# dkogan/horizonator

Measured on AMD Instinct MI355X. Metric: panorama Mpix/s (360deg, 16k-wide, 7x7 SRTM3 tiles), higher is better.
Workload: dtype f32

## Files before the change

### horizonator_amd/_lib.py

```python
import ctypes as C
import os

_HERE = os.path.dirname(os.path.abspath(__file__))
LIB_PATH = os.environ.get("HORIZONATOR_AMD_LIB") or os.path.join(_HERE, "libhorizonator.so")
DEMGEN_PATH = os.path.join(_HERE, "libhzdemgen.so")
SELFTEST_PATH = os.path.join(_HERE, "libhorizonator_selftest.so")

MAX_NDEMS_IJ = 4


class DemContext(C.Structure):
    _fields_ = [
        ("dems", (C.c_void_p * MAX_NDEMS_IJ) * MAX_NDEMS_IJ),
        ("mmap_sizes", (C.c_size_t * MAX_NDEMS_IJ) * MAX_NDEMS_IJ),
        ("mmap_fd", (C.c_int * MAX_NDEMS_IJ) * MAX_NDEMS_IJ),
        ("origin_dem_lon_lat", C.c_int * 2),
        ("origin_dem_cellij", C.c_int * 2),
        ("Ndems_ij", C.c_int * 2),
        ("radius_cells", C.c_int),
        ("cells_per_deg", C.c_int),
    ]


class _Offscreen(C.Structure):
    _fields_ = [
        ("inited", C.c_bool),
        ("frameBufID", C.c_uint32),
        ("renderBufID", C.c_uint32),
        ("depthBufID", C.c_uint32),
        ("width", C.c_int),
        ("height", C.c_int),
    ]


class Context(C.Structure):
    _fields_ = (
        [("Ntriangles", C.c_int), ("render_texture", C.c_bool), ("use_glut", C.c_bool),
         ("glut_window", C.c_int)]
        + [(name, C.c_int32) for name in (
            "uniform_aspect", "uniform_az_deg0", "uniform_az_deg1",
            "uniform_viewer_cell_i", "uniform_viewer_cell_j", "uniform_viewer_z",
            "uniform_viewer_lat", "uniform_cos_viewer_lat",
            "uniform_texturemap_lon0", "uniform_texturemap_lon1",
            "uniform_texturemap_dlat0", "uniform_texturemap_dlat1", "uniform_texturemap_dlat2",
            "uniform_znear", "uniform_zfar", "uniform_znear_color", "uniform_zfar_color")]
        + [("program", C.c_uint32), ("viewer_lat", C.c_float), ("viewer_lon", C.c_float),
           ("dems", DemContext), ("offscreen", _Offscreen)]
    )


class View(C.Structure):
    _fields_ = [(n, C.c_float) for n in (
        "viewer_cell_i", "viewer_cell_j", "viewer_z", "cos_viewer_lat", "deg_per_cell",
        "az_deg0", "az_deg1", "aspect", "znear", "zfar", "znear_color", "zfar_color")]


class Options(C.Structure):
    _fields_ = [(n, C.c_int) for n in (
        "serial", "rounds", "near_cells", "coarse_depth", "tiles", "tile_list", "adapt", "adapt_hi", "pretest_march",
        "worklists", "fast_math", "resolve_clears", "queue_capacity", "host_dense", "host_sectors", "host_times", "vertex_cache")]


class Times(C.Structure):
    _fields_ = [(n, C.c_float) for n in ("clear_ms", "raster_ms", "big_ms", "resolve_ms", "total_ms", "near_ms")]


class Window(C.Structure):
    _fields_ = [("cells_per_deg", C.c_int), ("radius_cells", C.c_int),
                ("origin_tile", C.c_int * 2), ("origin_cell", C.c_int * 2)]


class TexParams(C.Structure):
    _fields_ = [(n, C.c_float) for n in ("viewer_lat_rad", "origin_cell_lon_deg", "origin_cell_lat_deg",
                                         "lon0", "lon1", "dlat0", "dlat1", "dlat2")] + \
               [(n, C.c_int32) for n in ("ntiles_x", "ntiles_y", "lowest_x", "lowest_y", "tex_w", "tex_h")]


RASTER_AUTO, RASTER_SCATTER, RASTER_MARCH = 0, 1, 2

_lib = None
_selftest = None


def load():
    global _lib
    if _lib is None:
        _lib = _open(LIB_PATH, selftest=os.path.basename(LIB_PATH) == os.path.basename(SELFTEST_PATH))
    return _lib


def load_selftest():
    global _selftest
    if _selftest is None:
        _selftest = _open(SELFTEST_PATH, selftest=True)
    return _selftest


def _open(path, selftest):
    if not os.path.exists(path):
        raise ImportError(
            f"{path} is missing: build it with `make -C horizonator_amd/csrc` "
            "(or `python -c 'import __graft_entry__ as g; g.build()'`). "
            "horizonator_amd has no fallback implementation.")
    lib = C.CDLL(path, mode=C.RTLD_GLOBAL if not selftest else C.RTLD_LOCAL)
    P = C.POINTER
    ctxp = P(Context)
    f, i, b, d = C.c_float, C.c_int, C.c_bool, C.c_double
    vp = C.c_void_p

    def sig(name, res, *args):
        fn = getattr(lib, name)
        fn.restype = res
        fn.argtypes = list(args)

    sig("horizonator_init", b, ctxp, f, f, P(f), i, i, i, f, b, b, b,
        C.c_char_p, C.c_char_p, C.c_char_p, C.c_char_p, b)
    sig("horizonator_deinit", None, ctxp)
    sig("horizonator_resized", b, ctxp, i, i)
    sig("horizonator_pan_zoom", b, ctxp, f, f)
    sig("horizonator_move", b, ctxp, P(f), f, f)
    sig("horizonator_set_zextents", b, ctxp, f, f, f, f)
    sig("horizonator_redraw", b, ctxp)
    sig("horizonator_pick", b, ctxp, P(f), P(f), i, i)
    sig("horizonator_render_offscreen", b, ctxp, vp, vp)
    sig("horizonator_x_from_az", b, P(d), P(d), d, d, d, i)
    sig("horizonator_project", b, P(d), P(d), P(d), d, d, d, d, d, d, d, d, d, i, i)
    sig("horizonator_unproject", b, P(f), P(f), i, i, d, d, d, d, d, d, d, i, i)

    sig("horizonator_dem_init", b, P(DemContext), f, f, i, f, C.c_char_p, b)
    sig("horizonator_dem_deinit", None, P(DemContext))
    sig("horizonator_dem_sample", C.c_int16, P(DemContext), i, i)
    sig("horizonator_dem_bounds_latlon_deg", None, P(DemContext), P(f), P(f), P(f), P(f))

    sig("horizonator_amd_get_window", b, ctxp, P(Window))
    sig("horizonator_amd_init_from_mosaic", b, ctxp, f, f, P(f), i, i, P(Window), vp)
    sig("horizonator_amd_render", b, ctxp, vp, vp, vp, vp)
    sig("horizonator_amd_render_device", b, ctxp, vp, vp, vp, vp)
    sig("horizonator_amd_render_batch", b, ctxp, i, vp, vp, vp, vp, vp)
    sig("horizonator_amd_render_packed", b, ctxp, vp)
    sig("horizonator_amd_resolve_packed", b, ctxp, vp, i, i, i, vp, vp)
    sig("horizonator_amd_resolve_packed_strips", b, ctxp, i, vp, i, vp, vp, vp, vp)
    sig("horizonator_amd_render_sparse", b, ctxp, vp, i)
    sig("horizonator_amd_resolve_sparse_strips", b, ctxp, i, vp, i, vp, vp, vp, vp)
    sig("horizonator_amd_sync", b, ctxp)
    sig("horizonator_amd_texture_layout", b, ctxp, P(i), P(i), P(i), P(i))
    sig("horizonator_amd_set_texture", b, ctxp, vp)
    sig("horizonator_amd_set_sector", b, ctxp, i, i)
    sig("horizonator_amd_set_raster", b, ctxp, i)
    sig("horizonator_amd_set_profiling", b, ctxp, b)
    sig("horizonator_amd_render_begin", b, ctxp, vp, vp)
    sig("horizonator_amd_render_end", b, ctxp)
    sig("horizonator_amd_get_options", b, ctxp, P(Options))
    sig("horizonator_amd_set_options", b, ctxp, P(Options))
    sig("horizonator_amd_last_times", b, ctxp, P(Times))
    sig("horizonator_amd_get_view", b, ctxp, P(View))
    sig("horizonator_amd_device", vp, ctxp)
    sig("horizonator_amd_get_mosaic", b, ctxp, vp)
    sig("horizonator_amd_build_id", C.c_char_p)
    sig("horizonator_amd_link_cells_size", b, ctxp, i, i, i, P(i), P(i))
    sig("horizonator_amd_link_cells", b, ctxp, i, i, i, vp, vp)
    sig("horizonator_amd_poi_visibility", b, ctxp, i, vp, i, vp, vp, vp)

    sig("hz_hip_device_count", i)
    sig("hz_hip_create", vp, i, i, i, i)
    sig("hz_hip_destroy", None, vp)
    sig("hz_hip_upload_mosaic", i, vp, vp)
    sig("hz_hip_download_mosaic", i, vp, vp)
    sig("hz_hip_ingest_tiles", i, vp, vp, i, i, i, i, i)
    sig("hz_hip_set_sector", i, vp, i, i)
    sig("hz_hip_set_raster", i, vp, i)
    sig("hz_hip_set_profiling", i, vp, i)
    sig("hz_hip_get_options", i, vp, P(Options))
    sig("hz_hip_set_options", i, vp, P(Options))
    sig("hz_hip_set_texture", i, vp, P(TexParams), vp)
    sig("hz_hip_pack", i, vp, vp)
    sig("hz_hip_resolve_packed", i, vp, P(View), vp, vp, i, i, i, vp, vp)
    sig("hz_hip_pack_sparse", i, vp, vp, i)
    sig("hz_hip_resolve_sparse", i, vp, P(View), vp, vp, i, i, i, vp, vp)
    sig("hz_hip_resolve_sparse_strips", i, vp, P(View), vp, i, vp, i, vp, vp, vp, vp)
    sig("hz_hip_draw", i, vp, P(View))
    sig("hz_hip_resolve", i, vp, P(View), vp, vp, vp, vp, vp)
    sig("hz_hip_resolve_to_host", i, vp, P(View), vp, vp, vp, vp, vp)
    sig("hz_hip_render_to_host", i, vp, P(View), vp, vp, vp, vp, vp)
    sig("hz_hip_host_begin", i, vp, P(View), vp, vp, vp, vp, vp)
    sig("hz_hip_host_end", i, vp)
    sig("hz_hip_host_prepare", i, vp, i, i, i, i, vp)
    sig("hz_hip_read_depth", i, vp, i, i, P(C.c_uint32))
    sig("hz_hip_link_cells", i, vp, P(View), vp, vp, vp, vp, d, d, d, i, i, i, i, vp, vp)
    sig("hz_hip_poi_visibility", i, vp, P(View), vp, i, vp, i, vp, vp, vp)
    sig("hz_hip_sync", i, vp)
    sig("hz_hip_last_times", i, vp, P(Times))
    sig("hz_hip_stream", vp, vp)
    sig("hz_hip_wait_outputs", i, vp, vp)
    sig("hz_hip_wait_for", i, vp, vp)
    sig("horizonator_amd_stream_waits_for_outputs", b, ctxp, vp)
    sig("horizonator_amd_waits_for_stream", b, ctxp, vp)
    sig("hz_hip_last_plan", i, vp, vp)
    sig("hz_hip_last_queue_counts", i, vp, vp)
    sig("hz_hip_last_error", C.c_char_p)
    if selftest:
        sig("hz_hip_check_fastmath", i, i, i, C.c_uint64, C.c_uint64, P(C.c_uint64), vp)
        sig("hz_hip_check_exactness", i, i, i, C.c_uint64, C.c_uint64, i, i, i, i, P(C.c_uint64))
        sig("hz_hip_debug_bigqueue", i, vp, i, vp, i, vp)
        sig("hz_hip_debug_wave_timing", i, vp, P(View), vp, C.c_size_t, vp)
        sig("hz_hip_debug_worklist", C.c_long, i, i, i, P(View), i, i, i, vp, C.c_size_t)
    return lib


DECLARED_SYMBOLS = [
    "horizonator_init", "horizonator_deinit", "horizonator_resized", "horizonator_pan_zoom",
    "horizonator_move", "horizonator_set_zextents", "horizonator_redraw", "horizonator_pick",
    "horizonator_render_offscreen", "horizonator_x_from_az", "horizonator_project",
    "horizonator_unproject",
    "horizonator_dem_init", "horizonator_dem_deinit", "horizonator_dem_sample",
    "horizonator_dem_bounds_latlon_deg",
    "horizonator_amd_get_window", "horizonator_amd_init_from_mosaic",
    "horizonator_amd_render", "horizonator_amd_render_device", "horizonator_amd_render_batch",
    "horizonator_amd_render_packed", "horizonator_amd_resolve_packed",
    "horizonator_amd_resolve_packed_strips", "horizonator_amd_render_sparse",
    "horizonator_amd_resolve_sparse_strips",
    "horizonator_amd_sync", "horizonator_amd_stream_waits_for_outputs", "horizonator_amd_waits_for_stream", "horizonator_amd_texture_layout", "horizonator_amd_set_texture",
    "horizonator_amd_set_sector", "horizonator_amd_set_raster", "horizonator_amd_set_profiling",
    "horizonator_amd_get_options", "horizonator_amd_set_options", "horizonator_amd_render_begin", "horizonator_amd_render_end",
    "horizonator_amd_last_times", "horizonator_amd_get_view", "horizonator_amd_device",
    "horizonator_amd_get_mosaic", "horizonator_amd_link_cells_size", "horizonator_amd_link_cells",
    "horizonator_amd_poi_visibility", "horizonator_amd_build_id",
    "hz_hip_device_count", "hz_hip_create", "hz_hip_destroy", "hz_hip_upload_mosaic",
    "hz_hip_download_mosaic", "hz_hip_ingest_tiles", "hz_hip_set_sector", "hz_hip_set_raster",
    "hz_hip_set_profiling", "hz_hip_get_options", "hz_hip_set_options", "hz_hip_set_texture", "hz_hip_pack", "hz_hip_resolve_packed", "hz_hip_pack_sparse", "hz_hip_resolve_sparse", "hz_hip_resolve_sparse_strips", "hz_hip_draw", "hz_hip_resolve", "hz_hip_resolve_to_host", "hz_hip_render_to_host", "hz_hip_host_begin", "hz_hip_host_end", "hz_hip_host_prepare",
    "hz_hip_read_depth", "hz_hip_link_cells", "hz_hip_poi_visibility", "hz_hip_sync", "hz_hip_last_times", "hz_hip_stream", "hz_hip_wait_outputs", "hz_hip_wait_for", "hz_hip_last_plan", "hz_hip_last_queue_counts", "hz_hip_last_error",
]
SELFTEST_SYMBOLS = ["hz_hip_check_fastmath", "hz_hip_check_exactness", "hz_hip_debug_bigqueue", "hz_hip_debug_wave_timing",
                    "hz_hip_debug_worklist"]


def load_demgen():
    if not os.path.exists(DEMGEN_PATH):
        raise ImportError(f"{DEMGEN_PATH} is missing: build it with `make -C horizonator_amd/csrc`")
    lib = C.CDLL(DEMGEN_PATH)
    lib.hz_demgen_write_region.restype = C.c_int
    lib.hz_demgen_write_region.argtypes = [C.c_char_p] + [C.c_int] * 6
    lib.hz_demgen_write_tile.restype = C.c_int
    lib.hz_demgen_write_tile.argtypes = [C.c_char_p] + [C.c_int] * 4
    lib.hz_demgen_tile_values.restype = None
    lib.hz_demgen_tile_values.argtypes = [C.c_void_p] + [C.c_int] * 4
    return lib
```

### horizonator_amd/csrc/hz_context.cpp

```cpp
#include "hz_dev.h"

#include <time.h>

thread_local char hz_g_last_error[512];
extern "C" const char* hz_hip_last_error(void) { return g_last_error; }


static int env_int(const char* name, int dflt) { const char* e = getenv(name); return e ? atoi(e) : dflt; }
static hz_options_t default_options(void)
{
    hz_options_t o;
    o.serial         = 0;
    o.rounds         = 0;
    o.near_cells     = -1;
    o.coarse_depth   = -1;
    o.tiles          = -1;
    o.tile_list      = 0;
    o.adapt          = 1;
    o.adapt_hi       = -1;
    o.pretest_march  = -1;
    o.worklists      = 1;
    o.fast_math      = 1;
    o.resolve_clears = 1;
    o.queue_capacity = 0;
    o.host_dense     = 0;
    o.host_sectors   = 0;
    o.host_times     = 0;
    o.vertex_cache   = 1;
    return o;
}
hz_options_t hz_options_from_env(void)
{
    hz_options_t o = default_options();
    o.serial         = env_int("HZ_SERIAL", o.serial) != 0;
    if(getenv("HZ_TWO_PASS")) o.rounds = env_int("HZ_TWO_PASS", 0) != 0 ? 2 : 1;
    o.near_cells     = env_int("HZ_NEAR_CELLS", o.near_cells);
    if(getenv("HZ_HIZ")) o.coarse_depth = env_int("HZ_HIZ", 0) != 0;
    o.tiles          = env_int("HZ_TILES", o.tiles);
    o.tile_list      = env_int("HZ_TILE_LIST", o.tile_list);
    o.adapt          = env_int("HZ_ADAPT", o.adapt);
    o.adapt_hi       = env_int("HZ_ADAPT_HI", o.adapt_hi);
    if(getenv("HZ_PRETEST_MARCH")) o.pretest_march = env_int("HZ_PRETEST_MARCH", 0) != 0;
    o.worklists      = env_int("HZ_NO_WORKLIST", 0) == 0;
    o.fast_math      = env_int("HZ_NO_FAST_MATH", 0) == 0;
    o.resolve_clears = env_int("HZ_RESOLVE_CLEARS", o.resolve_clears) != 0;
    o.queue_capacity = env_int("HZ_QUEUE_CAPACITY", o.queue_capacity);
    o.host_dense     = env_int("HZ_HOST_DENSE", o.host_dense) != 0;
    o.host_sectors   = env_int("HZ_HOST_SECTORS", o.host_sectors);
    o.host_times     = env_int("HZ_HOST_TIMES", o.host_times) != 0;
    o.vertex_cache   = env_int("HZ_VERTEX_CACHE", o.vertex_cache) != 0;
    return o;
}
#ifdef HZ_EXPERIMENTS
static hz_experiments_t experiments_from_env(void)
{
    hz_experiments_t e = { env_int("HZ_MARCH_DEBUG", 0), env_int("HZ_EXP_FB_MARCH", 0), env_int("HZ_EXP_FB_BIG", 0) };
    return e;
}
#endif
extern "C" int hz_hip_device_count(void)
{
    int n = 0;
    if(hipGetDeviceCount(&n) != hipSuccess) return 0;
    return n;
}

hipError_t hz_sync_all(hz_dev_t* d)
{
    hipError_t rc = hipSuccess;
    hipStream_t all[4] = { d->stream, d->nstream, d->qstream, d->rstream };
    for(int k=0; k<4; k++)
        if(all[k]) { const hipError_t e = hipStreamSynchronize(all[k]); if(e != hipSuccess) rc = e; }
    return rc;
}

extern "C" void hz_hip_destroy(hz_dev_t* d)
{
    if(!d) return;
    hz_device_guard device_guard_(d->device);
    (void)hz_sync_all(d);
    (void)hipFree(d->d_mosaic);
    for(int i=0; i<HZ_NFB; i++) { (void)hipFree(d->d_fbs[i]); (void)hipFree(d->d_touched[i]); }
    for(int i=0; i<2*HZ_NFB; i++)
    {
        (void)hipFree(d->d_bigrec_s[i]);
        (void)hipFree(d->d_bigitem_s[i]);
        (void)hipFree(d->d_midrec_s[i]);
        (void)hipFree(d->d_clip_s[i]);
        (void)hipFree(d->d_big_counters_s[i]);
        (void)hipFree(d->tiles_s[i].cursor); (void)hipFree(d->tiles_s[i].pairs); (void)hipFree(d->tiles_s[i].state); (void)hipFree(d->tiles_s[i].busy);
    }
    if(d->ev_marched) (void)hipEventDestroy(d->ev_marched);
    if(d->ev_near)    (void)hipEventDestroy(d->ev_near);
    for(int i=0; i<HZ_NFB; i++) (void)hipFree(d->d_hiz[i]);
    for(int c=0; c<HZ_LIST_CACHE; c++)
        for(int k=0; k<HZ_NLISTS; k++)
        {
            hz_worklists_t& wl = d->list_cache[c];
            (void)hipFree(wl.d_items[k]);
            for(int t=0; t<2; t++)
            {
                if(wl.h_items[k][t])   (void)hipHostFree(wl.h_items[k][t]);
                if(wl.ev_copied[k][t]) (void)hipEventDestroy(wl.ev_copied[k][t]);
            }
        }
    delete d->list_scratch; delete d->list_scratch2;
    (void)hipFree(d->d_texels);
    (void)hipFree(d->d_tanel);
    free(d->h_tanel);
    hz_hostpath_destroy(d);
    (void)hipFree(d->vc.d_polar);
    if(d->vc.ev_filled) (void)hipEventDestroy(d->vc.ev_filled);
    for(int k=0; k<10; k++) if(d->ev[k]) (void)hipEventDestroy(d->ev[k]);
    for(int k=0; k<HZ_NFB; k++) { if(d->adapt.ev[k]) (void)hipEventDestroy(d->adapt.ev[k]); if(d->adapt.h_counts[k]) (void)hipHostFree(d->adapt.h_counts[k]); }
    if(d->ev_drawn)   (void)hipEventDestroy(d->ev_drawn);
    for(int i=0; i<HZ_NFB; i++) if(d->ev_free[i]) (void)hipEventDestroy(d->ev_free[i]);
    if(d->ev_readers) (void)hipEventDestroy(d->ev_readers);
    if(d->ev_tanel)   (void)hipEventDestroy(d->ev_tanel);
    if(d->rstream && d->rstream != d->stream) (void)hipStreamDestroy(d->rstream);
    if(d->qstream && d->qstream != d->stream) (void)hipStreamDestroy(d->qstream);
    if(d->nstream && d->nstream != d->stream) (void)hipStreamDestroy(d->nstream);

    if(d->stream) (void)hipStreamDestroy(d->stream);
    free(d);
}

int hz_tile_bins(hz_dev_t* d, int set)
{
    tl_bins_t& tb = d->tiles_s[set];
    if(tb.cursor) return 0;
    if(d->tiles_unavailable) return 1;
    const size_t ntiles = (size_t)((d->W + TL_W-1)/TL_W)*((d->H + TL_H-1)/TL_H);
    hipError_t e = hipMalloc(&tb.pairs, ntiles*TL_LIST*sizeof(unsigned int));
    if(e == hipSuccess) e = hipMalloc(&tb.state, 2*sizeof(unsigned int));
    if(e == hipSuccess) e = hipMalloc(&tb.busy, TL_UNITS_PER_TILE*ntiles*sizeof(unsigned int));
    if(e == hipSuccess) e = hipMalloc(&tb.cursor, ntiles*sizeof(unsigned int));
    if(e != hipSuccess)
    {
        (void)hipGetLastError();
        (void)hipFree(tb.pairs); (void)hipFree(tb.state); (void)hipFree(tb.busy); (void)hipFree(tb.cursor);
        tb.pairs = tb.state = tb.busy = tb.cursor = NULL;
        d->tiles_unavailable = 1;
        return 1;
    }
    return 0;
}

mr_queue_t hz_queue_set(const hz_dev_t* d, int k)
{
    const bool first_round = k >= HZ_NFB;
    mr_queue_t q = { d->d_bigrec_s[k], d->d_bigitem_s[k], d->d_midrec_s[k], d->d_clip_s[k], d->d_big_counters_s[k],
                     first_round ? d->near_bigrec_capacity  : d->bigrec_capacity,
                     first_round ? d->near_bigitem_capacity : d->bigitem_capacity,
                     first_round ? 0u : d->midrec_capacity,
                     first_round ? d->near_clip_capacity : d->clip_capacity };
    return q;
}


static int create_impl(hz_dev_t* d)
{
    hz_stopwatch sw("HZ_INIT_TIMES");
    HZ_ON_DEVICE(d);
    sw.lap("first HIP call (runtime, device)");
    d->env = hz_options_from_env();
#ifdef HZ_EXPERIMENTS
    d->exp = experiments_from_env();
#endif
    d->list_scratch = new std::vector<uint32_t>();
    d->list_scratch2 = new std::vector<uint32_t>();
    d->lists = &d->list_cache[0];
    HZ_CHECK(hipStreamCreateWithFlags(&d->stream, hipStreamNonBlocking));
    if(d->env.serial) d->rstream = d->stream;
    else HZ_CHECK(hipStreamCreateWithFlags(&d->rstream, hipStreamNonBlocking));
    HZ_CHECK(hipEventCreateWithFlags(&d->ev_drawn,   hipEventDisableTiming));
    for(int i=0; i<HZ_NFB; i++) HZ_CHECK(hipEventCreateWithFlags(&d->ev_free[i], hipEventDisableTiming));
    HZ_CHECK(hipEventCreateWithFlags(&d->ev_readers, hipEventDisableTiming));
    HZ_CHECK(hipEventCreateWithFlags(&d->ev_tanel,   hipEventDisableTiming));
    HZ_CHECK(hipMalloc(&d->d_mosaic, (size_t)d->N*d->N*sizeof(int16_t)));
    sw.lap("streams, events, mosaic");
    d->seg_stride = (d->W + HZ_SEG-1) / HZ_SEG;
    for(int i=0; i<HZ_NFB; i++)
    {
        HZ_CHECK(hipMalloc(&d->d_fbs[i], (size_t)d->W*d->H*sizeof(unsigned long long)));
        HZ_CHECK(hipMemsetAsync(d->d_fbs[i], 0xFF, (size_t)d->W*d->H*sizeof(unsigned long long), d->rstream));
        HZ_CHECK(hipMalloc(&d->d_touched[i], (size_t)d->seg_stride*d->H));
        HZ_CHECK(hipMemsetAsync(d->d_touched[i], 0, (size_t)d->seg_stride*d->H, d->rstream));
        HZ_CHECK(hipEventRecord(d->ev_free[i], d->rstream));
        d->fb_used[i] = 0;
    }
    d->fbi = HZ_NFB-1; d->d_fb = d->d_fbs[HZ_NFB-1];
    sw.lap("framebuffers");
    {
        const size_t per16 = (size_t)d->W*d->H/16;
        unsigned int rec = per16 > (1u<<24) ? (1u<<24) : per16 < (1u<<15) ? (1u<<15) : (unsigned int)per16;
        d->bigrec_capacity  = rec;
        d->bigitem_capacity = 2*rec;
        d->midrec_capacity  = rec;
        d->clip_capacity    = rec;
        const size_t r = (size_t)(d->env.near_cells > HZ_NEAR_CELLS_MAX ? d->env.near_cells : HZ_NEAR_CELLS_MAX);
        const size_t near_tris = 2*(2*r + 2)*(2*r + 2*MR_COLS);
        d->near_bigrec_capacity  = near_tris < rec ? (unsigned int)near_tris : rec;
        d->near_bigitem_capacity = 2*rec;
        d->near_clip_capacity    = d->near_bigrec_capacity;
        if(d->env.queue_capacity > 0)
            d->bigrec_capacity = d->bigitem_capacity = d->midrec_capacity = d->clip_capacity =
            d->near_bigrec_capacity = d->near_bigitem_capacity = d->near_clip_capacity = (unsigned int)d->env.queue_capacity;
    }
    if(d->env.serial) d->qstream = d->nstream = d->stream;
    else
    {
        HZ_CHECK(hipStreamCreateWithFlags(&d->qstream, hipStreamNonBlocking));
        HZ_CHECK(hipStreamCreateWithFlags(&d->nstream, hipStreamNonBlocking));
    }
    HZ_CHECK(hipEventCreateWithFlags(&d->ev_marched, hipEventDisableTiming));
    HZ_CHECK(hipEventCreateWithFlags(&d->ev_near,    hipEventDisableTiming));
    for(int i=0; i<2*HZ_NFB; i++)
    {
        const mr_queue_t q = hz_queue_set(d, i);
        HZ_CHECK(hipMalloc(&d->d_bigrec_s[i],  (size_t)q.bigrec_capacity*sizeof(hz_bigrec_t)));
        HZ_CHECK(hipMalloc(&d->d_bigitem_s[i], (size_t)q.bigitem_capacity*sizeof(hz_bigitem_t)));
        if(q.midrec_capacity) HZ_CHECK(hipMalloc(&d->d_midrec_s[i], (size_t)q.midrec_capacity*sizeof(hz_rec_t)));
        HZ_CHECK(hipMalloc(&d->d_clip_s[i],    (size_t)q.clip_capacity*sizeof(uint32_t)));
        HZ_CHECK(hipMalloc(&d->d_big_counters_s[i], HZ_NCOUNTERS*sizeof(unsigned int)));
        HZ_CHECK(hipMemset(d->d_big_counters_s[i], 0, HZ_NCOUNTERS*sizeof(unsigned int)));
        if(d->env.tiles > 0 && i >= HZ_NFB && hz_tile_bins(d, i) != 0) return -1;
    }
    sw.lap("queue sets");
    HZ_CHECK(hipEventRecord(d->ev_drawn, d->qstream));
    HZ_CHECK(hipMalloc(&d->d_tanel, (size_t)d->H*sizeof(float)));
    d->h_tanel = (float*)malloc((size_t)d->H*sizeof(float));
    d->tanel_resident = 0;
    for(int k=0; k<10; k++) HZ_CHECK(hipEventCreate(&d->ev[k]));
    for(int k=0; k<HZ_NFB; k++)
    {
        HZ_CHECK(hipHostMalloc((void**)&d->adapt.h_counts[k], 6*sizeof(unsigned int), hipHostMallocDefault));
        HZ_CHECK(hipEventCreateWithFlags(&d->adapt.ev[k], hipEventDisableTiming | hipEventReleaseToSystem));
    }
    sw.lap("the rest");
    return 0;
}

extern "C" hz_dev_t* hz_hip_create(int device, int N, int width, int height)
{
    if(N < 2 || width <= 0 || height <= 0)
    {
        snprintf(g_last_error, sizeof(g_last_error), "hz_hip_create: bad sizes N=%d W=%d H=%d", N, width, height);
        return NULL;
    }
    if((unsigned long long)width*(unsigned long long)height >= (1ull << 29))
    {
        snprintf(g_last_error, sizeof(g_last_error), "hz_hip_create: images of up to 2^29 pixels (%d x %d asked for)", width, height);
        fprintf(stderr, "hz_hip: %s\n", g_last_error);
        return NULL;
    }
    hz_dev_t* d = (hz_dev_t*)calloc(1, sizeof(*d));
    if(!d) return NULL;
    d->device = device; d->N = N; d->W = width; d->H = height;
    d->col0 = 0; d->col1 = width;
    d->raster = HZ_RASTER_AUTO;
    if(create_impl(d) != 0) { hz_hip_destroy(d); return NULL; }
    return d;
}

extern "C" int hz_hip_upload_mosaic(hz_dev_t* d, const int16_t* mosaic)
{
    HZ_ON_DEVICE(d);
    HZ_CHECK(hz_sync_all(d));
    HZ_CHECK(hipMemcpyAsync(d->d_mosaic, mosaic, (size_t)d->N*d->N*sizeof(int16_t), hipMemcpyHostToDevice, d->stream));
    HZ_CHECK(hipStreamSynchronize(d->stream));
    d->adapt.have_view = 0;
    d->vc.state = 0;
    return 0;
}

extern "C" int hz_hip_download_mosaic(hz_dev_t* d, int16_t* mosaic)
{
    HZ_ON_DEVICE(d);
    HZ_CHECK(hipMemcpyAsync(mosaic, d->d_mosaic, (size_t)d->N*d->N*sizeof(int16_t), hipMemcpyDeviceToHost, d->stream));
    HZ_CHECK(hipStreamSynchronize(d->stream));
    return 0;
}


extern "C" int hz_hip_set_sector(hz_dev_t* d, int col0, int col1)
{
    if(col0 < 0 || col1 > d->W || col0 >= col1)
    {
        snprintf(g_last_error, sizeof(g_last_error), "hz_hip_set_sector: bad sector [%d,%d) of %d", col0, col1, d->W);
        return -1;
    }
    d->col0 = col0; d->col1 = col1;
    return 0;
}

extern "C" int hz_hip_set_raster(hz_dev_t* d, int which)
{
    if(which < HZ_RASTER_AUTO || which > HZ_RASTER_MARCH) return -1;
    d->raster = which;
    return 0;
}

extern "C" int hz_hip_set_texture(hz_dev_t* d, const hz_texparams_t* params, const unsigned char* texels_bgr)
{
    HZ_ON_DEVICE(d);
    if(params == NULL) { d->tex_on = 0; return 0; }
    if(params->tex_w <= 0 || params->tex_h <= 0 || params->ntiles_x <= 0 || params->ntiles_y <= 0)
    {
        snprintf(g_last_error, sizeof(g_last_error), "hz_hip_set_texture: empty texture");
        return -1;
    }
    if(texels_bgr != NULL)
    {
        const size_t n = (size_t)params->tex_w*params->tex_h;
        uint32_t* packed = (uint32_t*)malloc(n*sizeof(uint32_t));
        if(!packed) { snprintf(g_last_error, sizeof(g_last_error), "hz_hip_set_texture: out of memory"); return -1; }
        for(size_t k=0; k<n; k++)
            packed[k] = (uint32_t)texels_bgr[3*k] | ((uint32_t)texels_bgr[3*k+1] << 8) | ((uint32_t)texels_bgr[3*k+2] << 16);
        HZ_CHECK(hipStreamSynchronize(d->stream));
        HZ_CHECK(hipStreamSynchronize(d->rstream));
        (void)hipFree(d->d_texels); d->d_texels = NULL;
        hipError_t e = hipMalloc(&d->d_texels, n*sizeof(uint32_t));
        if(e == hipSuccess) e = hipMemcpy(d->d_texels, packed, n*sizeof(uint32_t), hipMemcpyHostToDevice);
        free(packed);
        HZ_CHECK(e);
    }
    else if(d->d_texels == NULL || params->tex_w != d->tex.tex_w || params->tex_h != d->tex.tex_h)
    {
        snprintf(g_last_error, sizeof(g_last_error), "hz_hip_set_texture: no texture of that size is resident");
        return -1;
    }
    d->tex = *params;
    d->tex_on = 1;
    return 0;
}

extern "C" int hz_hip_set_profiling(hz_dev_t* d, int on) { d->profiling = on; return 0; }

extern "C" int hz_hip_get_options(hz_dev_t* d, hz_options_t* o)
{
    if(!d || !o) return -1;
    *o = d->env;
    return 0;
}
extern "C" int hz_hip_set_options(hz_dev_t* d, const hz_options_t* o)
{
    if(!d || !o) return -1;
    HZ_ON_DEVICE(d);
    HZ_CHECK(hz_sync_all(d));
    const int serial = d->env.serial, queue_capacity = d->env.queue_capacity;
    d->env = *o;
    d->env.serial = serial; d->env.queue_capacity = queue_capacity;
    for(int c=0; c<HZ_LIST_CACHE; c++) d->list_cache[c].valid = 0;
    d->adapt.have_view = 0;
    return 0;
}
extern "C" void* hz_hip_stream(hz_dev_t* d) { return (void*)d->rstream; }

extern "C" int hz_hip_wait_outputs(hz_dev_t* d, void* stream)
{
    HZ_ON_DEVICE(d);
    HZ_CHECK(hipEventRecord(d->ev_tanel, d->rstream));
    HZ_CHECK(hipStreamWaitEvent((hipStream_t)stream, d->ev_tanel, 0));
    return 0;
}

extern "C" int hz_hip_wait_for(hz_dev_t* d, void* stream)
{
    HZ_ON_DEVICE(d);
    HZ_CHECK(hipEventRecord(d->ev_tanel, (hipStream_t)stream));
    HZ_CHECK(hipStreamWaitEvent(d->rstream, d->ev_tanel, 0));
    return 0;
}

extern "C" int hz_hip_last_queue_counts(hz_dev_t* d, unsigned int* out)
{
    if(!d || !out) return -1;
    out[0] = (unsigned int)d->adapt.seen_reach; out[1] = d->adapt.seen_records; out[2] = d->adapt.seen_items; out[3] = (unsigned int)d->adapt.long_reach;
    return 0;
}

extern "C" int hz_hip_last_plan(hz_dev_t* d, int* out)
{
    if(!d || !out) return -1;
    for(int k=0; k<5; k++) out[k] = d->last_plan[k];
    return 0;
}


extern "C" int hz_hip_sync(hz_dev_t* d)
{
    HZ_ON_DEVICE(d);
    HZ_CHECK(hz_sync_all(d));
    return 0;
}

extern "C" int hz_hip_last_times(hz_dev_t* d, hz_times_t* t)
{
    memset(t, 0, sizeof(*t));
    if(!d->have_times) return -1;
    HZ_ON_DEVICE(d);
    HZ_CHECK(hz_sync_all(d));
    HZ_CHECK(hipEventElapsedTime(&t->clear_ms,  d->ev[0], d->ev[1]));
    HZ_CHECK(hipEventElapsedTime(&t->near_ms,   d->ev[7], d->ev[6]));
    HZ_CHECK(hipEventElapsedTime(&t->raster_ms, d->ev[9], d->ev[2]));
    HZ_CHECK(hipEventElapsedTime(&t->big_ms,    d->ev[8], d->ev[3]));
    if(d->have_times == 2)
        HZ_CHECK(hipEventElapsedTime(&t->resolve_ms, d->ev[4], d->ev[5]));
    t->total_ms = t->clear_ms + t->near_ms + t->raster_ms + t->big_ms + t->resolve_ms;
    return 0;
}
```

### horizonator_amd/csrc/hz_dev.h

```cpp
#pragma once

#include <hip/hip_runtime_api.h>

#include <math.h>
#include <stdio.h>
#include <stdlib.h>
#include <string.h>
#include <time.h>

#include <vector>

#include "hz_hip.h"
#include "hz_types.h"
#include "hz_launch.h"


extern thread_local char hz_g_last_error[512];
#define g_last_error hz_g_last_error

#define HZ_CHECK(call)                                                        \
    do {                                                                      \
        hipError_t e_ = (call);                                               \
        if(e_ != hipSuccess)                                                  \
        {                                                                     \
            snprintf(g_last_error, sizeof(g_last_error), "%s:%d %s -> %s",    \
                     __FILE__, __LINE__, #call, hipGetErrorString(e_));       \
            fprintf(stderr, "hz_hip: %s\n", g_last_error);                    \
            return -1;                                                        \
        }                                                                     \
    } while(0)

struct hz_device_guard
{
    int prev, dev; bool ok;
    explicit hz_device_guard(int device) : prev(-1), dev(device), ok(true)
    {
        if(hipGetDevice(&prev) != hipSuccess) prev = -1;
        if(prev != dev)
        {
            const hipError_t e = hipSetDevice(dev);
            if(e != hipSuccess)
            {
                ok = false;
                snprintf(g_last_error, sizeof(g_last_error), "hipSetDevice(%d) -> %s", dev, hipGetErrorString(e));
                fprintf(stderr, "hz_hip: %s\n", g_last_error);
            }
        }
    }
    ~hz_device_guard() { if(ok && prev >= 0 && prev != dev) (void)hipSetDevice(prev); }
};
#define HZ_ON_DEVICE(d) hz_device_guard device_guard_((d)->device); if(!device_guard_.ok) return -1

#ifdef HZ_EXPERIMENTS
struct hz_experiments_t { int march_debug, exp_fb_march, exp_fb_big; };
#endif

struct hz_listkey_t
{
    hz_view_t view; int col0, col1, two_pass, near_x0, near_x1, near_j0, near_j1, far_rows;
};
#define HZ_NLISTS 2
struct hz_worklists_t
{
    uint32_t*    d_items[HZ_NLISTS];
    uint32_t*    h_items[HZ_NLISTS][2];
    size_t       cap[HZ_NLISTS];
    unsigned int n[HZ_NLISTS];
    hipEvent_t   ev_copied[HZ_NLISTS][2];
    int          turn[HZ_NLISTS];
    int          valid;
    unsigned int last_used;
    hz_listkey_t key;
};
#define HZ_LIST_CACHE 8

struct hz_dev
{
    int device;
    hz_options_t env;
#ifdef HZ_EXPERIMENTS
    hz_experiments_t exp;
#endif
    int N, W, H;
    int col0, col1;
    int raster;
    int profiling;
    hz_worklists_t list_cache[HZ_LIST_CACHE];
    hz_worklists_t* lists;
    unsigned int lists_clock;
    std::vector<uint32_t>* list_scratch;
    std::vector<uint32_t>* list_scratch2;
    struct { unsigned long long* d_cycles; size_t capacity; unsigned int grid_x, grid_y; } wave_timing;

    hipStream_t stream, rstream;
    hipEvent_t  ev_drawn, ev_free[HZ_NFB], ev_readers, ev_tanel;
    int16_t*            d_mosaic;
    unsigned long long* d_fbs[HZ_NFB];
    size_t              fb_used[HZ_NFB];
    int                 fbi;
    unsigned long long* d_fb;
    unsigned char*      d_touched[HZ_NFB];
    int                 seg_stride;
    hipStream_t         qstream, nstream;
    hipEvent_t          ev_marched, ev_near;
    uint32_t*           d_hiz[HZ_NFB];
    int                 hiz_unavailable;
    int                 tiles_unavailable;
    struct
    {
        unsigned int* h_counts[HZ_NFB];
        hipEvent_t    ev[HZ_NFB];
        int           pending[HZ_NFB], long_of[HZ_NFB], reach_of[HZ_NFB];
        unsigned int  serial_of[HZ_NFB];
        hz_view_t     view; int col0, col1, have_view;
        unsigned int  serial;
        unsigned int  items_short;
        int           tried_long;
        int           long_reach;
        int           seen_reach; unsigned int seen_records, seen_items;
    } adapt;
    struct { hz_polar_t* d_polar; hz_xform_t key; int state ; int unavailable; hipEvent_t ev_filled;
             int same_draw;      } vc;
    int                 last_qshards_log2;
    int                 last_plan[5];
    int                 stream_reads_fb;
    hz_bigrec_t*        d_bigrec_s[2*HZ_NFB];
    hz_bigitem_t*       d_bigitem_s[2*HZ_NFB];
    hz_rec_t*           d_midrec_s[2*HZ_NFB];
    uint32_t*           d_clip_s[2*HZ_NFB];
    unsigned int*       d_big_counters_s[2*HZ_NFB];
    unsigned int        bigrec_capacity, bigitem_capacity, midrec_capacity, clip_capacity;
    unsigned int        near_bigrec_capacity, near_bigitem_capacity, near_clip_capacity;
    tl_bins_t           tiles_s[2*HZ_NFB];
    hz_view_t           last_view;
    int                 have_view;
    int                 fb_consumed;
    float*              d_tanel;
    float*              h_tanel;
    int                 tanel_resident;

    struct hz_hoststate* host;

    uint32_t*      d_texels;
    hz_texparams_t tex;
    int            tex_on;

    hipEvent_t ev[10];
    int        have_times;
    hz_times_t times;
};

#define HZ_NEAR_PX            20.0f
#define HZ_TWO_ROUNDS_MIN_PIX 6.0e6
#define HZ_TILES_MIN_PX       35.0f
#define HZ_HIZ_MIN_PX         25.0f



struct hz_stopwatch
{
    bool on; timespec t0;
    explicit hz_stopwatch(const char* var) : on(getenv(var) && atoi(getenv(var)) != 0) { clock_gettime(CLOCK_MONOTONIC, &t0); }
    void lap(const char* what)
    {
        if(!on) return;
        timespec t1; clock_gettime(CLOCK_MONOTONIC, &t1);
        fprintf(stderr, "hz_hip init: %-34s %8.2f ms\n", what, 1e3*(double)(t1.tv_sec - t0.tv_sec) + 1e-6*(double)(t1.tv_nsec - t0.tv_nsec));
        t0 = t1;
    }
};


hz_options_t hz_options_from_env(void);
mr_queue_t   hz_queue_set(const hz_dev_t* d, int k);
int          hz_tile_bins(hz_dev_t* d, int set);
hipError_t   hz_sync_all(hz_dev_t* d);
hz_params_t  hz_make_params(const hz_dev_t* d, const hz_view_t* v);
int          hz_plan_rounds(const hz_dev_t* d, const hz_view_t* view, hz_params_t& p);
mr_zones_t   hz_make_zones(const hz_params_t& p, bool near_first);
bool         hz_azimuths_of_columns(const hz_params_t& p, double* a0, double* a1);
void         hz_list_items(const hz_params_t& p, const mr_zones_t& zn, double a0, double a1, std::vector<uint32_t>& out, bool every_strip = false);
void         hz_list_rounds(const hz_params_t& p, const mr_zones_t& zn, double a0, double a1, bool one_round,
                            std::vector<uint32_t>* first, std::vector<uint32_t>& second, bool every_strip = false);
int          hz_draw_impl(hz_dev_t* d, const hz_view_t* view);
int          hz_fb_refill(hz_dev_t* d);
int          hz_fb_mark_consumed(hz_dev_t* d);
int          hz_upload_tanel(hz_dev_t* d, const float* tanel);
int          hz_rstream_after_draw(hz_dev_t* d);
int          hz_resolve_impl(hz_dev_t* d, const hz_view_t* view, const float* tanel,
                             unsigned char* bgr, float* ranges, int32_t* index, uint32_t* z24, int nbands, hipEvent_t* ev_band, int* band_rows);
void         hz_hostpath_destroy(hz_dev_t* d);
int          hz_gpu_numa_node(const hz_dev_t* d);
void         hz_hostpath_landing(hz_dev_t* d, unsigned char** pinned, size_t* bytes);
```

### horizonator_amd/csrc/hz_fast.h

```cpp
#pragma once

#include "hz_num.h"

#ifdef __HIPCC__

#define HZF_LO 9.31322575e-10f
#define HZF_HI 1073741824.0f

__device__ static inline int hzf_in_range(float x) { const float a = hz_abs(x); return a >= HZF_LO && a <= HZF_HI; }

__device__ static inline float hzf_refined_rcp(float c)
{
    const float r = __builtin_amdgcn_rcpf(c);
    const float e = __builtin_fmaf(-c, r, 1.0f);
    return __builtin_fmaf(e, r, r);
}
__device__ static inline float hzf_div_by(float a, float c, float rr)
{
    float q = a*rr;
    float e = __builtin_fmaf(-c, q, a);
    q = __builtin_fmaf(e, rr, q);
    e = __builtin_fmaf(-c, q, a);
    return __builtin_fmaf(e, rr, q);
}
__device__ static inline float hzf_div(float a, float b) { return hzf_div_by(a, b, hzf_refined_rcp(b)); }
__device__ static inline float hzf_rcp(float b)          { return hzf_refined_rcp(b); }
__device__ static inline float hzf_div_by_two_pi(float a, float rr)
{
    const float q = a*rr;
    const float e = __builtin_fmaf(-HZ_TWO_PI, q, a);
    return __builtin_fmaf(e, rr, q);
}
__device__ static inline float hzf_fold_to_unit(float t) { return (1.0f < t) ? hzf_rcp(t) : t; }

__device__ static inline float hzf_sqrt(float x)
{
    const float y = __builtin_amdgcn_rsqf(x);
    const float s = x*y;
    const float h = 0.5f*y;
    const float r = __builtin_fmaf(-s, s, x);
    return __builtin_fmaf(r, h, s);
}

typedef struct { float rr_two_pi, rr_zrange, rr_crange, zrange, crange; } hzf_const_t;

__device__ static inline hzf_const_t hzf_setup(const hz_xform_t* u)
{
    hzf_const_t c;
    c.zrange = u->zfar - u->znear;
    c.crange = u->zfar_color - u->znear_color;
    float two_pi = HZ_TWO_PI;
    asm volatile("" : "+v"(two_pi));
    c.rr_two_pi = hzf_refined_rcp(two_pi);
    c.rr_zrange = hzf_refined_rcp(c.zrange);
    c.rr_crange = hzf_refined_rcp(c.crange);
    return c;
}

template<bool XPOS>
__device__ static inline float hzf_atan2_r(float y, float x, float rcp)
{
    const bool  flip = XPOS ? false : (0.f >= x);
    const float ax   = hz_abs(x);
    const float s    = flip ? ax : y;
    const float sot  = s * rcp;
    const float tn   = (ax == hz_abs(y)) ? 1.0f : hz_abs(sot);

    const float u  = hzf_fold_to_unit(tn);
    const float u2 = u*u;
    const float u3 = u2*u;
    const float u5 = u3*u2;
    const float u7 = u5*u2;
    const float u9 = u7*u2;
    float p = u*0.9999793128310355f + u3*-0.3326756418091246f;
    p = p + u5*0.1938924977115610f;
    p = p + u7*-0.1173503194786851f;
    p = p + u9*0.0536813784310406f;
    p = p + (u9*-0.0121323213173444f)*u2;
    const float a   = (1.0f < tn) ? ((p*-2.0f + HZ_HALF_PI) + p) : p;
    const float arc = flip ? (HZ_HALF_PI + a) : a;
    const uint32_t sign = ((uint32_t)__float_as_int(y) | (uint32_t)__float_as_int(rcp)) & 0x80000000u;
    return __int_as_float((int)((uint32_t)__float_as_int(arc) | sign));
}
template<bool XPOS>
__device__ static inline float hzf_atan2(float y, float x)
{
    const float t = (XPOS ? false : (0.f >= x)) ? y : hz_abs(x);
    return hzf_atan2_r<XPOS>(y, x, hzf_rcp(t));
}

__device__ static inline hz_polar_t hzf_polar_en_r(const hz_xform_t* u, float e, float n, float fz, float rcp_az)
{
    hz_polar_t q;
    const float h = fz - u->viewer_z;
    const float nn = n*n, ee = e*e;
    q.d_ne  = hzf_sqrt(nn + ee);
    q.az    = hzf_atan2_r<false>(e, n, rcp_az);
    q.el    = hzf_atan2<true>(h, q.d_ne);
    q.d_enh = hzf_sqrt(h*h + nn + ee);
    return q;
}
__device__ static inline hz_polar_t hzf_polar_en(const hz_xform_t* u, float e, float n, float fz)
{
    return hzf_polar_en_r(u, e, n, fz, hzf_rcp((0.f >= n) ? e : hz_abs(n)));
}
__device__ static inline hz_vertex_t hzf_finish(const hz_xform_t* u, const hzf_const_t* c, hz_polar_t q)
{
    hz_vertex_t v;
    const float d = hzf_div_by_two_pi(q.az + -u->az_center, c->rr_two_pi);
    v.x = (HZ_TWO_PI*(d - hz_roundeven(d))) * u->az_ndc_per_rad;
    v.y = q.el * u->aspect * u->az_ndc_per_rad;
    v.z = hzf_div_by(q.d_enh - u->znear, c->zrange, c->rr_zrange) * 2.0f + -1.0f;

    const float r = hzf_div_by(q.d_ne - u->znear_color, c->crange, c->rr_crange);
    v.red = hz_min(hz_max(r, 0.0f), 1.0f);
    return v;
}
__device__ static inline hz_vertex_t hzf_transform_en(const hz_xform_t* u, const hzf_const_t* c, float e, float n, float fz)
{
    return hzf_finish(u, c, hzf_polar_en(u, e, n, fz));
}
__device__ static inline hz_vertex_t hzf_transform_en_r(const hz_xform_t* u, const hzf_const_t* c, float e, float n, float fz, float rcp_az)
{
    return hzf_finish(u, c, hzf_polar_en_r(u, e, n, fz, rcp_az));
}

#endif

HZ_HD int hzf_draw_ok(const hz_xform_t* u)
{
    const float lo = 9.31322575e-10f, hi = 1073741824.0f;
    const float vz = hz_abs(u->viewer_z), ce = hz_abs(u->az_center);
    const float zr = hz_abs(u->zfar - u->znear), cr = hz_abs(u->zfar_color - u->znear_color);
    if(!(vz == 0.0f || (vz >= 0.015625f && vz <= 536870912.0f))) return 0;
    if(!(ce == 0.0f || (ce >= 8.8817842e-16f && ce <= 1048576.0f))) return 0;
    if(!(u->znear >= lo && u->znear <= hi && hz_abs(u->zfar) >= lo && hz_abs(u->zfar) <= hi && zr >= lo && zr <= hi)) return 0;
    if(!(hz_abs(u->znear_color) >= lo && hz_abs(u->znear_color) <= hi &&
         hz_abs(u->zfar_color) >= lo && hz_abs(u->zfar_color) <= hi && cr >= lo && cr <= hi)) return 0;
    if(!(hz_abs(u->aspect) <= hi && hz_abs(u->az_ndc_per_rad) <= hi)) return 0;
    return 1;
}
```

### horizonator_amd/csrc/hz_ingest.cpp

```cpp
#include "hz_dev.h"
#include "hz_pool.h"

extern "C" int hz_hip_ingest_tiles(hz_dev_t* d, const unsigned char* const* tiles,
                                   int ntx, int nty, int cpd, int oc_x, int oc_y)
{
    HZ_ON_DEVICE(d);
    const int nt = ntx*nty;
    const size_t tile_bytes = (size_t)(cpd+1)*(cpd+1)*2;
    if(nt <= 0 || !tiles) { snprintf(g_last_error, sizeof(g_last_error), "hz_hip_ingest_tiles: no tiles"); return -1; }
    HZ_CHECK(hz_sync_all(d));
    int npresent = 0;
    for(int k=0; k<nt; k++) if(tiles[k]) npresent++;
    unsigned char* d_raw = NULL;
    unsigned char** d_ptrs = NULL;
    unsigned char* own_stage = NULL;
    std::vector<unsigned char*> h_ptrs((size_t)nt, (unsigned char*)NULL);
    int rc = -1;
    hipEvent_t ev[3] = { NULL, NULL, NULL };
    do {
        if(npresent && hipMalloc(&d_raw, (size_t)npresent*tile_bytes) != hipSuccess) { snprintf(g_last_error, sizeof(g_last_error), "hz_hip_ingest_tiles: no device memory for %d tiles", npresent); break; }
        if(hipMalloc(&d_ptrs, (size_t)nt*sizeof(*d_ptrs)) != hipSuccess) break;
        for(int k=0, at=0; k<nt; k++) if(tiles[k]) h_ptrs[(size_t)k] = d_raw + (size_t)(at++)*tile_bytes;
        unsigned char* stage = NULL; size_t stage_bytes = 0;
        hz_hostpath_landing(d, &stage, &stage_bytes);
        if(stage_bytes < ((size_t)3 << 20))
        {
            stage_bytes = (size_t)24 << 20;
            if(hipHostMalloc((void**)&own_stage, stage_bytes, hipHostMallocDefault) != hipSuccess) { snprintf(g_last_error, sizeof(g_last_error), "hz_hip_ingest_tiles: no pinned memory"); break; }
            stage = own_stage;
        }
        size_t piece = stage_bytes/3 & ~(size_t)4095;
        if(piece > ((size_t)64 << 20)) piece = (size_t)64 << 20;
        bool ok = true;
        for(int k=0; k<3 && ok; k++) ok = hipEventCreateWithFlags(&ev[k], hipEventDisableTiming) == hipSuccess;
        if(!ok) break;
        hz_copy_pool* pool = copy_pool(hz_gpu_numa_node(d));
        const size_t total = (size_t)npresent*tile_bytes;
        std::vector<const unsigned char*> src;
        for(int k=0; k<nt; k++) if(tiles[k]) src.push_back(tiles[k]);
        size_t turn = 0;
        for(size_t off = 0; off < total && ok; off += piece, turn++)
        {
            const size_t n = total - off < piece ? total - off : piece;
            unsigned char* buf = stage + (turn % 3)*piece;
            if(turn >= 3) ok = hipEventSynchronize(ev[turn % 3]) == hipSuccess;
            if(!ok) break;
            hz_copy_pool::batch_t copied = { 0 };
            for(size_t o = off; o < off + n; )
            {
                const size_t t = o/tile_bytes, in = o - t*tile_bytes;
                const size_t len = tile_bytes - in < off + n - o ? tile_bytes - in : off + n - o;
                pool->push(&copied, buf + (o - off), src[t] + in, len, (size_t)1 << 20);
                o += len;
            }
            pool->wait(&copied);
            ok = hipMemcpyAsync(d_raw + off, buf, n, hipMemcpyHostToDevice, d->stream) == hipSuccess
              && hipEventRecord(ev[turn % 3], d->stream) == hipSuccess;
        }
        if(!ok) { snprintf(g_last_error, sizeof(g_last_error), "hz_hip_ingest_tiles: tile upload failed"); break; }
        if(hipMemcpyAsync(d_ptrs, h_ptrs.data(), (size_t)nt*sizeof(*d_ptrs), hipMemcpyHostToDevice, d->stream) != hipSuccess) break;
        dim3 grid((d->N + 255)/256, d->N);
        hzk_ingest(grid, dim3(256), d->stream, (const unsigned char* const*)d_ptrs, d->d_mosaic, d->N, ntx, nty, cpd, oc_x, oc_y);
        if(hipGetLastError() != hipSuccess) break;
        if(hipStreamSynchronize(d->stream) != hipSuccess) break;
        d->adapt.have_view = 0;
        d->vc.state = 0;
        rc = 0;
    } while(0);
    (void)hipStreamSynchronize(d->stream);
    for(int k=0; k<3; k++) if(ev[k]) (void)hipEventDestroy(ev[k]);
    (void)hipFree(d_raw); (void)hipFree(d_ptrs);
    if(own_stage) (void)hipHostFree(own_stage);
    (void)hipGetLastError();
    return rc;
}
```

### horizonator_amd/csrc/hz_k_march.h

```cpp
#pragma once


#define MR_CAP    128
#define MR_RSLOTS 4
#define MR_FIELDS 6

struct mr_lds_t
{
    uint32_t rows[MR_RSLOTS][MR_FIELDS][64];
    uint32_t ids[MR_CAP];
    uint32_t clip[64];
    uint32_t nclip;
};

__device__ static inline void mr_clip_flush(mr_lds_t& L, const mr_queue_t& q, int lane)
{
    const unsigned int nclip = (unsigned int)__builtin_amdgcn_readfirstlane((int)L.nclip);
    if(!nclip) return;
    uint32_t base = 0;
    if(lane == 0) base = atomicAdd(&q.counters[4], nclip);
    base = (uint32_t)__builtin_amdgcn_readfirstlane((int)base);
    if((unsigned int)lane < nclip)
    {
        const uint32_t at = base + (uint32_t)lane;
        if(at < q.clip_capacity) q.clip[at] = L.clip[lane];
    }
    __syncthreads();
    if(lane == 0) L.nclip = 0;
    __syncthreads();
}
__device__ static inline void mr_clip_note(mr_lds_t& L, const mr_queue_t& q, bool want, uint32_t prim, int lane)
{
    const unsigned long long m = __ballot(want);
    if(!m) return;
    const unsigned int n = (unsigned int)__popcll(m);
    unsigned int nclip = (unsigned int)__builtin_amdgcn_readfirstlane((int)L.nclip);
    if(nclip + n > 64u) { mr_clip_flush(L, q, lane); nclip = 0; }
    if(want) L.clip[nclip + (unsigned int)__popcll(m & ((1ull << lane) - 1ull))] = prim;
    __syncthreads();
    if(lane == 0) L.nclip = nclip + n;
    __syncthreads();
}

__device__ static inline void mr_store_row(mr_lds_t& L, int slot, int lane, const hz_wvert_t& v)
{
    L.rows[slot][0][lane] = __float_as_uint(v.wx);  L.rows[slot][1][lane] = __float_as_uint(v.wy);
    L.rows[slot][2][lane] = __float_as_uint(v.zw);  L.rows[slot][3][lane] = __float_as_uint(v.red);
    L.rows[slot][4][lane] = (uint32_t)v.xs;         L.rows[slot][5][lane] = (uint32_t)v.ys;
}
__device__ static inline hz_wvert_t mr_load_vert(const mr_lds_t& L, int slot, int lane)
{
    hz_wvert_t v;
    v.xn  = 0.f;
    v.wx  = __uint_as_float(L.rows[slot][0][lane]); v.wy  = __uint_as_float(L.rows[slot][1][lane]);
    v.zw  = __uint_as_float(L.rows[slot][2][lane]); v.red = __uint_as_float(L.rows[slot][3][lane]);
    v.xs  = (int32_t)L.rows[slot][4][lane];         v.ys  = (int32_t)L.rows[slot][5][lane];
    v.cmask = 0;
    return v;
}

__device__ static inline hz_wvert_t mr_load_vert_pos(const mr_lds_t& L, int slot, int lane)
{
    hz_wvert_t v;
    v.xn  = 0.f; v.red = 0.f; v.cmask = 0;
    v.wx  = __uint_as_float(L.rows[slot][0][lane]); v.wy  = __uint_as_float(L.rows[slot][1][lane]);
    v.zw  = __uint_as_float(L.rows[slot][2][lane]);
    v.xs  = (int32_t)L.rows[slot][4][lane];         v.ys  = (int32_t)L.rows[slot][5][lane];
    return v;
}


__device__ static inline int32_t mr_from_east(int32_t v)
{
    return __builtin_amdgcn_update_dpp(0, v, 0x130 , 0xF, 0xF, true);
}
__device__ static inline float mr_from_east(float v)
{
    return __int_as_float(__builtin_amdgcn_update_dpp(0, __float_as_int(v), 0x130, 0xF, 0xF, true));
}



__device__ static inline int32_t hz_imin(int32_t a, int32_t b) { return a < b ? a : b; }
__device__ static inline int32_t hz_imax(int32_t a, int32_t b) { return a > b ? a : b; }

struct mr_rowstate_t
{
    float    xn;
    int32_t  xs, ys;
    uint32_t cmask;
    uint32_t c, f1;
    uint32_t e_c, e_f1;
    uint32_t h_c, h_f1;
    int32_t  h_dx, h_dy;
};

__device__ static inline hz_wvert_t mr_window(const hz_vertex_t& vtx, const hz_params_t& p, bool* in_volume, bool* in_guard)
{
    hz_wvert_t cur;
    cur.xn  = vtx.x;
    cur.wx  = vtx.x*p.halfW + p.halfW;
    cur.wy  = vtx.y*p.halfH + p.halfH;
    cur.zw  = vtx.z*0.5f + 0.5f;
    cur.red = vtx.red;
    const float fxw = cur.wx - 0.5f, fyw = cur.wy - 0.5f;
    *in_guard  = hz_abs(fxw) <= HZ_GUARD_PX && hz_abs(fyw) <= HZ_GUARD_PX;
    *in_volume = __builtin_fmaxf(__builtin_fmaxf(hz_abs(vtx.x), hz_abs(vtx.y)), hz_abs(vtx.z)) <= 1.0f;
    cur.xs = (int32_t)hz_roundeven(fxw*256.f);
    cur.ys = (int32_t)hz_roundeven(fyw*256.f);
    cur.cmask = 0;
    return cur;
}
__device__ static inline void mr_window_flags(hz_wvert_t& cur, const hz_vertex_t& vtx, bool in_guard)
{
    cur.cmask = hz_clip_mask(vtx.x, vtx.y, vtx.z);
    if(!in_guard) { cur.xs = HZ_OUTSIDE_GUARD; cur.ys = 0; }
}

__device__ static inline uint32_t mr_pk_min(uint32_t a, uint32_t b)
{
    typedef unsigned short u16x2 __attribute__((ext_vector_type(2)));
    return __builtin_bit_cast(uint32_t, __builtin_elementwise_min(__builtin_bit_cast(u16x2, a), __builtin_bit_cast(u16x2, b)));
}
__device__ static inline uint32_t mr_pk_max(uint32_t a, uint32_t b)
{
    typedef unsigned short u16x2 __attribute__((ext_vector_type(2)));
    return __builtin_bit_cast(uint32_t, __builtin_elementwise_max(__builtin_bit_cast(u16x2, a), __builtin_bit_cast(u16x2, b)));
}
__device__ static inline bool mr_pk_lt(uint32_t a, uint32_t b)
{
    typedef unsigned short u16x2 __attribute__((ext_vector_type(2)));
    const u16x2 x = __builtin_bit_cast(u16x2, a), y = __builtin_bit_cast(u16x2, b);
    return x.x < y.x && x.y < y.y;
}
__device__ static inline uint32_t mr_from_east_u(uint32_t v) { return (uint32_t)mr_from_east((int32_t)v); }

__device__ static inline mr_rowstate_t mr_rowstate_of(const hz_wvert_t& cur, const hz_params_t& p)
{
    mr_rowstate_t now;
    now.xn = cur.xn; now.xs = cur.xs; now.ys = cur.ys; now.cmask = cur.cmask;
    const uint32_t c_x  = (uint32_t)((cur.xs + (HZ_SUBPIXEL_ONE-1)) >> HZ_SUBPIXEL_BITS), c_y  = (uint32_t)((cur.ys + (HZ_SUBPIXEL_ONE-1)) >> HZ_SUBPIXEL_BITS);
    const uint32_t f1_x = (uint32_t)((cur.xs + HZ_SUBPIXEL_ONE) >> HZ_SUBPIXEL_BITS),     f1_y = (uint32_t)((cur.ys + HZ_SUBPIXEL_ONE) >> HZ_SUBPIXEL_BITS);
    now.c  = mr_pk_max(c_x  | (c_y  << 16), (uint32_t)p.col0);
    now.f1 = mr_pk_min(f1_x | (f1_y << 16), (uint32_t)p.col1 | ((uint32_t)p.H << 16));
    now.e_c  = mr_from_east_u(now.c);
    now.e_f1 = mr_from_east_u(now.f1);
    now.h_c  = mr_pk_min(now.e_c,  now.c);
    now.h_f1 = mr_pk_max(now.e_f1, now.f1);
    now.h_dx = (int32_t)((uint32_t)mr_from_east(cur.xs) - (uint32_t)cur.xs);
    now.h_dy = (int32_t)((uint32_t)mr_from_east(cur.ys) - (uint32_t)cur.ys);
    return now;
}

__device__ static inline bool mr_simple_cull(const mr_rowstate_t& prev, const mr_rowstate_t& now, bool has_cell,
                                             const hz_params_t& p, bool* keep0, bool* keep1)
{
    const int32_t d01x = (int32_t)((uint32_t)now.xs - (uint32_t)prev.xs);
    const int32_t d01y = (int32_t)((uint32_t)now.ys - (uint32_t)prev.ys);
    const int32_t d11x = (int32_t)((uint32_t)d01x + (uint32_t)now.h_dx);
    const int32_t d11y = (int32_t)((uint32_t)d01y + (uint32_t)now.h_dy);
    const int32_t d10x = prev.h_dx, d10y = prev.h_dy;
    const int32_t lo = hz_imin(hz_imin(d01x, d11x), d10x), hi = hz_imax(hz_imax(d01x, d11x), d10x);
    if(__any(has_cell && !(lo > -p.quad_max_dx && hi < p.quad_max_dx))) return false;
    const int64_t area0 = (int64_t)d11x*(int64_t)d01y - (int64_t)d01x*(int64_t)d11y;
    const int64_t area1 = (int64_t)d10x*(int64_t)d11y - (int64_t)d11x*(int64_t)d10y;
    const uint32_t c0 = mr_pk_min(now.h_c, prev.c),                 f0 = mr_pk_max(now.h_f1, prev.f1);
    const uint32_t c1 = mr_pk_min(now.e_c, prev.h_c), f1 = mr_pk_max(now.e_f1, prev.h_f1);
    const bool box0 = mr_pk_lt(c0, f0), box1 = mr_pk_lt(c1, f1);
    *keep0 = has_cell && area0 > 0 && box0;
    *keep1 = has_cell && area1 > 0 && box1;
    return true;
}

__device__ static void mr_distribute(const hz_rec_t& r, uint32_t npix, int lane,
                                     unsigned long long* fb, const hz_params_t& p)
{
    uint32_t done = 0;
    for(;;)
    {
        const bool more = npix > done;
        if(__popcll(__ballot(more)) < 32) break;
        if(more)
        {
            const int ry = (int)(((float)done + 0.5f) * r.inv_bw);
            const int rx = (int)done - ry*r.bw;
            hz_emit_rec<false>(fb, p, r, r.px0 + rx, r.py0 + ry);
            done++;
        }
    }

    const uint32_t rest  = npix > done ? npix - done : 0;
    const uint32_t incl  = mr_scan(rest, lane);
    const uint32_t excl  = incl - rest;
    const uint32_t total = (uint32_t)__builtin_amdgcn_readlane((int)incl, 63);
    for(uint32_t base = 0; base < total; base += 64)
    {
        const uint32_t it = base + lane;
        int lo = 0;
        #pragma unroll
        for(int step=32; step>=1; step>>=1)
        {
            const uint32_t v = __shfl(excl, lo + step);
            if(v <= it) lo += step;
        }
        hz_rec_t o;
        #pragma unroll
        for(int m=0; m<3; m++)
        {
            o.e.dx[m]  = __shfl(r.e.dx[m], lo);  o.e.ndy[m] = __shfl(r.e.ndy[m], lo);
            o.e.glo[m] = __shfl(r.e.glo[m], lo); o.e.ghi[m] = __shfl(r.e.ghi[m], lo);
        }
        o.z_org = __shfl(r.z_org, lo); o.dzdx = __shfl(r.dzdx, lo); o.dzdy = __shfl(r.dzdy, lo);
        o.r_org = __shfl(r.r_org, lo); o.drdx = __shfl(r.drdx, lo); o.drdy = __shfl(r.drdy, lo);
        o.px0 = __shfl(r.px0, lo); o.py0 = __shfl(r.py0, lo); o.bw = __shfl(r.bw, lo);
        o.inv_bw = __shfl(r.inv_bw, lo);
        o.prim = __shfl(r.prim, lo);
        const uint32_t oexcl = __shfl(excl, lo), odone = __shfl(done, lo);
        if(it < total)
        {
            const uint32_t local = it - oexcl + odone;
            const int ry = (int)(((float)local + 0.5f) * o.inv_bw);
            const int rx = (int)local - ry*o.bw;
            hz_emit_rec<false>(fb, p, o, o.px0 + rx, o.py0 + ry);
        }
    }
}

__global__ __launch_bounds__(64)
void k_mid(unsigned long long* __restrict__ fb, const hz_rec_t* __restrict__ midrec,
           const unsigned int* __restrict__ counters, unsigned int midrec_capacity, hz_params_t p)
{
    const int lane = threadIdx.x;
    const int sl = p.qshards_log2;
    unsigned int longest = 0;
    #pragma unroll
    for(int s=0; s<HZ_QSHARDS; s++) { const unsigned int* c = hz_qshard(counters, s) + 4; longest = max(longest, min(min(c[0], ~c[1]), HZ_QSHARD_ROOM(midrec_capacity, sl))); }
    const unsigned int n = ((longest + HZ_QBLOCK-1) & ~(unsigned int)(HZ_QBLOCK-1)) << sl;
    for(unsigned int base = blockIdx.x*64u; base < n; base += gridDim.x*64u)
    {
        hz_rec_t r = {};
        uint32_t npix = 0;
        const unsigned int g = base + lane, block = g >> HZ_QBLOCK_LOG2;
        const unsigned int* c = hz_qshard(counters, (int)(block & ((1u << sl) - 1u))) + 4;
        if(g < n && (((block >> sl) << HZ_QBLOCK_LOG2) | (g & (HZ_QBLOCK-1))) < min(min(c[0], ~c[1]), HZ_QSHARD_ROOM(midrec_capacity, sl)))
        {
            r = midrec[g];
            npix = __float_as_uint(r.inv_bw);
            r.inv_bw = 1.0f / (float)r.bw;
        }
        mr_distribute(r, npix, lane, fb, p);
    }
}

template<bool HIZ, bool SHARDS>
__device__ static void mr_flush(const mr_lds_t& L, unsigned int head, unsigned int n, int lane,
                                int jbeg, int i0,
                                unsigned long long* fb, const mr_queue_t& q, const hz_params_t& p,
                                unsigned int* dbg = nullptr)
{
    hz_rec_t r;
    uint32_t npix = 0;
    int bh = 0;
    bool live = (unsigned int)lane < n;
    const bool valid = live;
    const uint32_t id_own = L.ids[(head + lane) & (MR_CAP-1)];
    const uint32_t id = valid ? id_own : (uint32_t)__builtin_amdgcn_readlane((int)id_own, 0);
    const int t = id & 1, l = (id >> 1) & 63, rowoff = id >> 7;
    const int s0 = rowoff & (MR_RSLOTS-1), s1 = (rowoff+1) & (MR_RSLOTS-1);
    const int sa = s0,               la = l;
    const int sb = t == 0 ? s1 : s0, lb = l+1;
    const int sc = s1,               lc = t == 0 ? l : l+1;
    hz_wvert_t a = mr_load_vert_pos(L, sa, la);
    hz_wvert_t b = mr_load_vert_pos(L, sb, lb);
    hz_wvert_t c = mr_load_vert_pos(L, sc, lc);
    hz_box_t box;
    hz_tri_box(&box, &a, &b, &c, p.col0, p.col1-1, 0, p.H-1);
    if(p.early_z)
    {
        if(valid && box.px1 - box.px0 <= 3 && box.py1 - box.py0 <= 1)
        {
            const char* hi = (const char*)fb + 4;
            const uint32_t rowbytes = (uint32_t)p.SW*8u;
            const uint32_t o0 = (uint32_t)box.py0*rowbytes, o1 = box.py1 > box.py0 ? o0 + rowbytes : o0;
            const int c0 = box.px0 - p.col0, cl = box.px1 - p.col0;
            typedef uint32_t u3_t __attribute__((ext_vector_type(3)));
            const int ca = min(c0, p.SW - 2), cb = min(max(cl - 1, c0), p.SW - 2);
            const uint32_t ba = 8u*(uint32_t)ca, bb = 8u*(uint32_t)cb;
            const u3_t a0 = *(const u3_t*)(hi + (o0 + ba)), b0 = *(const u3_t*)(hi + (o0 + bb));
            const u3_t a1 = *(const u3_t*)(hi + (o1 + ba)), b1 = *(const u3_t*)(hi + (o1 + bb));
            const uint32_t zs = max(max(max(a0.x, a0.z), max(b0.x, b0.z)), max(max(a1.x, a1.z), max(b1.x, b1.z))) >> 8;
            if(hz_tri_hidden(&a, &b, &c, p.z_hide_k, zs)) live = false;
        }
        else if(HIZ && valid && p.hiz)
        {
            const int bw1 = box.px1 - box.px0, bh1 = box.py1 - box.py0;
            const bool lv1 = bw1 <= (1 << HIZ1_W_LOG2) && bh1 <= (1 << HIZ1_H_LOG2);
            if(lv1 || (bw1 <= (1 << HIZ2_W_LOG2) && bh1 <= (1 << HIZ2_H_LOG2)))
            {
                const uint32_t* t = lv1 ? p.hiz : hiz_level2(p);
                const int sx = lv1 ? HIZ1_W_LOG2 : HIZ2_W_LOG2, sy = lv1 ? HIZ1_H_LOG2 : HIZ2_H_LOG2;
                const uint32_t tw = (uint32_t)(lv1 ? hiz_w1(p.SW) : hiz_w2(p.SW));
                const uint32_t tx0 = (uint32_t)(box.px0 - p.col0) >> sx, tx1 = (uint32_t)(box.px1 - p.col0) >> sx;
                const uint32_t o0 = ((uint32_t)box.py0 >> sy)*tw, o1 = ((uint32_t)box.py1 >> sy)*tw;
                const uint32_t z00 = t[o0 + tx0], z01 = t[o0 + tx1], z10 = t[o1 + tx0], z11 = t[o1 + tx1];
                const uint32_t zs = max(max(z00, z01), max(z10, z11)) >> 8;
                if(hz_tri_hidden(&a, &b, &c, p.z_hide_k, zs)) live = false;
            }
        }
        if(dbg) { dbg[5] += (unsigned int)__popcll(__ballot(valid && !live)); }
        if(HZ_DEBUG(p) == 2) return;
        if(!__any(live))
        {
            if(dbg) { dbg[0] += 1; dbg[1] += n; }
            return;
        }
    }
    {
        a.red = __uint_as_float(L.rows[sa][3][la]);
        b.red = __uint_as_float(L.rows[sb][3][lb]);
        c.red = __uint_as_float(L.rows[sc][3][lc]);
        hz_tri_t tri;
        hz_tri_planes(&tri, &a, &b, &c);
        hz_rec_from_tri(r, tri);
        r.px0 = box.px0; r.bw = box.px1 - box.px0 + 1;
        r.py0 = box.py0; bh   = box.py1 - box.py0 + 1;
        r.prim = (uint32_t)(((size_t)(jbeg + rowoff)*(p.N-1) + (i0 + l))*2 + t);
        npix = live ? (uint32_t)r.bw*(uint32_t)bh : 0u;
        r.inv_bw = __all(npix <= 64u) ? __builtin_amdgcn_rcpf((float)r.bw) : 1.0f / (float)r.bw;
    }

    const bool is_big = live && npix > p.big_min;
    const unsigned long long bigmask = __ballot(is_big);
    if(dbg) { dbg[0] += 1; dbg[1] += n; dbg[2] += (unsigned int)__popcll(bigmask); }
    const unsigned long long t_app0 = (dbg && HZ_DEBUG(p) == 4) ? __builtin_amdgcn_s_memtime() : 0ull;
    if(bigmask)
    {
        uint32_t chunks = 0;
        if(is_big)
        {
            chunks = hz_big_chunks(r.bw, bh);
        }
        const uint32_t incl  = mr_scan(chunks, lane);
        const uint32_t total = (uint32_t)__builtin_amdgcn_readlane((int)incl, 63);
        const uint32_t nb    = (uint32_t)__popcll(bigmask);
        uint32_t rbase = 0, ibase = 0, ok = 0;
        const int sl = SHARDS ? HZ_QSHARDS_LOG2 : 0, shard = (int)((blockIdx.x + 5u*blockIdx.y) & ((1u << sl) - 1u));
        if(lane == 0)
        {
            ok = hz_queue_reserve(q, shard, sl, nb, total, &rbase, &ibase) ? 1u : 0u;
        }
        rbase = (uint32_t)__builtin_amdgcn_readfirstlane((int)rbase); ibase = (uint32_t)__builtin_amdgcn_readfirstlane((int)ibase); ok = (uint32_t)__builtin_amdgcn_readfirstlane((int)ok);
        if(is_big)
        {
            if(ok)
            {
                const uint32_t ri = HZ_QSLOT(rbase + (uint32_t)__popcll(bigmask & ((1ull << lane) - 1ull)), shard, sl);
                const uint32_t ii = ibase + (incl - chunks);
                q.bigrec[ri].r = r; q.bigrec[ri].bh = bh;
                for(uint32_t c2=0; c2<chunks; c2++) { const uint32_t g = HZ_QSLOT(ii + c2, shard, sl); q.bigitem[g].rec = ri; q.bigitem[g].chunk = c2; }
            }
            else
            {
                for(int py = r.py0; py < r.py0 + bh; py++)
                    for(int px = r.px0; px < r.px0 + r.bw; px++)
                        hz_emit_rec<true>(fb, p, r, px, py);
            }
            npix = 0;
        }
    }

    const bool is_mid = live && npix > p.inline_max;
    const unsigned long long midmask = __ballot(is_mid);
    if(dbg) { dbg[3] += (unsigned int)__popcll(midmask); }
    if(midmask)
    {
        const int slm = SHARDS ? HZ_QSHARDS_LOG2 : 0, mshard = (int)((blockIdx.x + 5u*blockIdx.y) & ((1u << slm) - 1u));
        unsigned int* const mc = hz_qshard(q.counters, mshard) + 4;
        uint32_t mbase = 0;
        if(lane == 0) mbase = atomicAdd(mc, (uint32_t)__popcll(midmask));
        mbase = (uint32_t)__builtin_amdgcn_readfirstlane((int)mbase);
        if(mbase + (uint32_t)__popcll(midmask) <= HZ_QSHARD_ROOM(q.midrec_capacity, slm))
        {
            if(is_mid)
            {
                hz_rec_t m = r;
                m.inv_bw = __uint_as_float(npix);
                q.midrec[HZ_QSLOT(mbase + (uint32_t)__popcll(midmask & ((1ull << lane) - 1ull)), mshard, slm)] = m;
                npix = 0;
            }
        }
        else if(lane == 0) atomicMax(mc + 1, ~mbase);
    }

    if(dbg && HZ_DEBUG(p) == 4)
    {
        const unsigned long long t1 = __builtin_amdgcn_s_memtime();
        dbg[3] += (unsigned int)((t1 - t_app0) >> 4);
        mr_distribute(r, npix, lane, fb, p);
        dbg[4] += (unsigned int)((__builtin_amdgcn_s_memtime() - t1) >> 4);
        return;
    }
    if(dbg) { const uint32_t tot = (uint32_t)__builtin_amdgcn_readlane((int)mr_scan(npix, lane), 63); dbg[4] += tot; }
    mr_distribute(r, npix, lane, fb, p);
}

#ifdef MR_WAVES_PER_EU
#define MR_OCCUPANCY __attribute__((amdgpu_waves_per_eu(MR_WAVES_PER_EU, MR_WAVES_PER_EU)))
#elif defined(MR_VGPRS)
#define MR_OCCUPANCY __attribute__((amdgpu_num_vgpr(MR_VGPRS)))
#else
#define MR_OCCUPANCY
#endif
template<bool COUNTERS, bool HIZ, bool VCACHE, bool SHARDS>
__global__ __launch_bounds__(64) MR_OCCUPANCY
void k_march(const int16_t* __restrict__ mosaic, unsigned long long* __restrict__ fb,
             mr_queue_t q, mr_zones_t zn, hz_params_t p)
{
    __shared__ mr_lds_t L;
    const unsigned long long t_start = COUNTERS ? __builtin_amdgcn_s_memtime() : 0ull;
    unsigned int dbgv[6] = {0,0,0,0,0,0};
    unsigned int* dbg = COUNTERS ? dbgv : nullptr;

    const int lane = threadIdx.x;
    int sx, seg;
    if(p.worklist)
    {
        const uint32_t item = p.worklist[blockIdx.x];
        sx = (int)(item & ((1u << MR_ITEM_SX_BITS) - 1u)); seg = (int)(item >> MR_ITEM_SX_BITS);
    }
    else { sx = (int)blockIdx.x + (p.pass == 1 ? p.near_x0 : 0); seg = (int)blockIdx.y; }
    const int i0   = sx*MR_COLS;
    const int i    = i0 + lane;
    int jbeg, jend;
    mr_segment_rows(zn, seg, &jbeg, &jend);
    if(p.pass)
    {
        const bool near = sx >= p.near_x0 && sx <= p.near_x1 && jbeg < p.near_j1 && jend > p.near_j0;
        if((p.pass == 1) != near) return;
    }
    const bool has_vertex = i < p.N;
    const bool has_cell   = lane < MR_COLS && i < p.N-1;
    const int  ic = has_vertex ? i : p.N-1;

    if(p.cull_strips)
    {
        const int ia = i0, ib = min(i0 + MR_COLS, p.N-1);
        const bool viewer_inside = p.u.viewer_cell_i >= (float)(ia-1) && p.u.viewer_cell_i <= (float)(ib+1) &&
                                   p.u.viewer_cell_j >= (float)(jbeg-1) && p.u.viewer_cell_j <= (float)(jend+1);
        if(!viewer_inside)
        {
            const hz_vertex_t v = hz_transform_en(&p.u, hz_east(&p.u, (float)((lane & 1) ? ib : ia)),
                                                  hz_north(&p.u, (float)((lane & 2) ? jend : jbeg)), 0.f);
            float xlo = 2.f, xhi = -2.f;
            #pragma unroll
            for(int c=0; c<4; c++)
            {
                const float xc = __builtin_bit_cast(float, __builtin_amdgcn_readlane(__builtin_bit_cast(int, v.x), c));
                xlo = hz_min(xlo, xc); xhi = hz_max(xhi, xc);
            }
            if(xhi - xlo <= 1.0f)
            {
                const float flo = (xlo*p.halfW + p.halfW) - 2.5f, fhi = (xhi*p.halfW + p.halfW) + 1.5f;
                if(fhi < (float)p.col0 || flo > (float)p.col1) return;
            }
        }
    }

    const float e = hz_east(&p.u, (float)ic);
    const float n_tab = hz_north(&p.u, (float)(jbeg + lane));
    auto north_of = [&](int rel) -> float
    {
        if(rel < 64) return __builtin_bit_cast(float, __builtin_amdgcn_readlane(__builtin_bit_cast(int, n_tab), rel));
        return hz_north(&p.u, (float)(jbeg + rel));
    };
    if(p.far_strips)
    {
        const int nrows = jend - jbeg;
        float nn = lane <= nrows ? n_tab*n_tab : __builtin_inff();
        if(nrows >= 64) { const float n64 = hz_north(&p.u, (float)(jbeg + 64)); nn = hz_min(nn, n64*n64); }
        #pragma unroll
        for(int m=32; m>=1; m>>=1) nn = hz_min(nn, __shfl_xor(nn, m));
        if(__all(nn + e*e > p.far_dd)) return;
    }

    const hzf_const_t fc = hzf_setup(&p.u);
    const bool fast_strip = p.fast_ok && __all(hzf_in_range(e));
    const unsigned long long fast_rows = __ballot(hzf_in_range(n_tab));
    const int  tab_rows   = min(jend - jbeg, 63);
    const bool rcp_south  = __all(lane > tab_rows || 0.f >= n_tab);
    const bool rcp_north  = __all(lane > tab_rows || !(0.f >= n_tab));
    const float rcp_tab   = VCACHE ? 0.f : hzf_rcp(rcp_south ? e : hz_abs(n_tab));

    unsigned int head = 0, count = 0;
    if(lane == 0) L.nclip = 0;
    __syncthreads();
    int first_row = 0;
    mr_rowstate_t prev = {};
    bool prev_simple = false;
    int16_t z_next = VCACHE ? (int16_t)0 : mosaic[(size_t)jbeg*p.N + ic];
    hz_polar_t q_next = {};
    if(VCACHE) q_next = p.vcache[(size_t)jbeg*p.N + ic];
    float n_cur = north_of(0);
    bool far_prev = true;
    bool far_cur  = __all(n_cur*n_cur + e*e > p.far_dd);
    for(int j = jbeg; j <= jend; j++)
    {
        const int rel = j - jbeg;
        const float z = (float)z_next;
        const hz_polar_t q_cur = q_next;
        if(j < jend)
        {
            if(VCACHE) q_next = p.vcache[(size_t)(j+1)*p.N + ic];
            else z_next = mosaic[(size_t)(j+1)*p.N + ic];
        }
        const float n_next   = (j == jend) ? 0.f : north_of(rel+1);
        const bool  far_next = (j == jend) || __all(n_next*n_next + e*e > p.far_dd);
        const bool  skip_row   = far_prev && far_cur && far_next;
        const bool  skip_cells = far_prev && far_cur;
        const float n = n_cur;
        n_cur = n_next; far_prev = far_cur; far_cur = far_next;
        if(skip_row) continue;

        const bool fast = fast_strip && (rel >= 64 ? hzf_in_range(n) : (int)((fast_rows >> rel) & 1ull));
        hz_vertex_t vtx;
        if(VCACHE) vtx = fast ? hzf_finish(&p.u, &fc, q_cur) : hz_finish(&p.u, q_cur);
        else if(fast)
        {
            float rcp_az;
            if(rel >= 64 || !(rcp_south || rcp_north)) rcp_az = hzf_rcp((0.f >= n) ? e : hz_abs(n));
            else if(rcp_south) rcp_az = rcp_tab;
            else rcp_az = __builtin_bit_cast(float, __builtin_amdgcn_readlane(__builtin_bit_cast(int, rcp_tab), rel));
            vtx = hzf_transform_en_r(&p.u, &fc, e, n, z, rcp_az);
#ifdef HZ_EXP_TRANSFORM_TWICE
            {
                float n2 = n; asm volatile("" : "+v"(n2));
                const hz_vertex_t v2 = hzf_transform_en_r(&p.u, &fc, e, n2, z, rcp_az);
                vtx.x = (v2.x == vtx.x) ? vtx.x : v2.y; vtx.y = (v2.y == vtx.y) ? vtx.y : v2.z;
                vtx.z = (v2.z == vtx.z) ? vtx.z : v2.x; vtx.red = (v2.red == vtx.red) ? vtx.red : v2.x;
            }
#endif
        }
        else vtx = hz_transform_en(&p.u, e, n, z);

        bool in_volume, in_guard;
        hz_wvert_t cur = mr_window(vtx, p, &in_volume, &in_guard);
        const bool cur_simple = __all(in_guard && in_volume);
        if(!cur_simple) mr_window_flags(cur, vtx, in_guard);

        if(count && first_row <= rel - MR_RSLOTS)
        {
            __syncthreads();
            mr_flush<HIZ, SHARDS>(L, head, count, lane, jbeg, i0, fb, q, p, dbg);
            __syncthreads();
            head = (head + count) & (MR_CAP-1);
            count = 0;
        }
        mr_store_row(L, rel & (MR_RSLOTS-1), lane, cur);

        const mr_rowstate_t now = mr_rowstate_of(cur, p);

        if(j > jbeg && !skip_cells)
        {
            bool keep0 = false, keep1 = false;
            if(cur_simple && prev_simple && mr_simple_cull(prev, now, has_cell, p, &keep0, &keep1))
            {
            }
            else
            {
                hz_wvert_t v00 = {}, v01 = {}, v10 = {}, v11 = {};
                v00.xn = prev.xn; v00.xs = prev.xs; v00.ys = prev.ys; v00.cmask = prev.cmask;
                v01.xn = cur.xn;  v01.xs = cur.xs;  v01.ys = cur.ys;  v01.cmask = cur.cmask;
                v10.xn = mr_from_east(prev.xn);
                v10.xs = (int32_t)((uint32_t)prev.xs + (uint32_t)prev.h_dx); v10.ys = (int32_t)((uint32_t)prev.ys + (uint32_t)prev.h_dy);
                v10.cmask = (uint32_t)mr_from_east((int32_t)prev.cmask);
                v11.xn = mr_from_east(cur.xn);
                v11.xs = (int32_t)((uint32_t)cur.xs + (uint32_t)now.h_dx);   v11.ys = (int32_t)((uint32_t)cur.ys + (uint32_t)now.h_dy);
                v11.cmask = (uint32_t)mr_from_east((int32_t)cur.cmask);
                hz_box_t box;
                const int verdict0 = has_cell ? hz_tri_cull(&box, &v00, &v11, &v01, p.col0, p.col1-1, 0, p.H-1) : HZ_TRI_DROP;
                const int verdict1 = has_cell ? hz_tri_cull(&box, &v00, &v10, &v11, p.col0, p.col1-1, 0, p.H-1) : HZ_TRI_DROP;
                const uint32_t prim0 = (uint32_t)(((size_t)(j-1)*(p.N-1) + i)*2);
                mr_clip_note(L, q, verdict0 == HZ_TRI_CLIP, prim0,   lane);
                mr_clip_note(L, q, verdict1 == HZ_TRI_CLIP, prim0+1, lane);
                keep0 = verdict0 == HZ_TRI_DRAW; keep1 = verdict1 == HZ_TRI_DRAW;
            }
            #pragma unroll
            for(int t=0; t<2; t++)
            {
                const bool keep = (t == 0 ? keep0 : keep1) && HZ_DEBUG(p) != 1;
                const unsigned long long m = __ballot(keep);
                if(m)
                {
                    if(count == 0) first_row = rel-1;
                    if(keep)
                    {
                        const unsigned int at = (head + count + (unsigned int)__popcll(m & ((1ull << lane) - 1ull))) & (MR_CAP-1);
                        L.ids[at] = ((uint32_t)(rel-1) << 7) | ((uint32_t)lane << 1) | (uint32_t)t;
                    }
                    count += (unsigned int)__popcll(m);
                    if(count >= 64)
                    {
                        __syncthreads();
                        mr_flush<HIZ, SHARDS>(L, head, 64, lane, jbeg, i0, fb, q, p, dbg);
                        head = (head + 64) & (MR_CAP-1);
                        count -= 64;
                        if(count) first_row = (int)(L.ids[head] >> 7);
                        __syncthreads();
                    }
                }
            }
        }
        prev = now; prev_simple = cur_simple;
    }
    if(count)
    {
        __syncthreads();
        mr_flush<HIZ, SHARDS>(L, head, count, lane, jbeg, i0, fb, q, p, dbg);
    }
    mr_clip_flush(L, q, lane);
    if(COUNTERS && p.wave_cycles && lane == 0)
    {
        unsigned long long* o = &p.wave_cycles[((size_t)blockIdx.y*gridDim.x + blockIdx.x)*4];
        o[0] = __builtin_amdgcn_s_memtime() - t_start;
        o[1] = ((unsigned long long)dbgv[0] << 32) | dbgv[1];
        o[2] = ((unsigned long long)dbgv[2] << 32) | dbgv[3];
        o[3] = ((unsigned long long)dbgv[5] << 32) | dbgv[4];
    }
}
```

### horizonator_amd/csrc/hz_kernels.hip

```cpp
#include <hip/hip_runtime.h>

#include <math.h>
#include <stdio.h>
#include <stdlib.h>
#include <string.h>

#include "hz_hip.h"
#include "hz_types.h"
#include "hz_fast.h"

#include "hz_k_common.h"
#include "hz_k_hiz.h"
#include "hz_k_scatter.h"
#include "hz_k_tile.h"
#include "hz_k_march.h"
#include "hz_k_resolve.h"
#include "hz_k_tell.h"
#include "hz_k_tex.h"


__global__ __launch_bounds__(256)
void k_ingest(const unsigned char* const* __restrict__ tiles, int16_t* __restrict__ mosaic,
              int N, int ntx, int nty, int cpd, int oc_x, int oc_y)
{
    const int i = blockIdx.x*blockDim.x + threadIdx.x;
    const int j = blockIdx.y;
    if(i >= N) return;
    int cx = i + oc_x, tx = cx / cpd; cx -= tx*cpd; if(cx == 0 && tx > 0) { tx--; cx = cpd; }
    int cy = j + oc_y, ty = cy / cpd; cy -= ty*cpd; if(cy == 0 && ty > 0) { ty--; cy = cpd; }
    int16_t z = -1;
    if(tx < ntx && ty < nty)
    {
        const unsigned char* t = tiles[tx + ty*ntx];
        if(t == NULL) z = 0;
        else
        {
            const size_t q = (size_t)cx + (size_t)(cpd - cy)*(size_t)(cpd+1);
            const unsigned short be = *(const unsigned short*)(t + 2*q);
            z = (int16_t)(unsigned short)((be << 8) | (be >> 8));
            if(z < 0) z = 0;
        }
    }
    mosaic[(size_t)j*N + i] = z;
}


__device__ static inline float hz_range_of(unsigned long long key, float tanel_row, float znear, float zfar)
{
    const uint32_t zi = (uint32_t)(key >> 40);
    if(zi == HZ_Z24_MAX) return -1.0f;
    const float depth = (float)((double)zi * (1.0/16777215.0));
    const float len   = depth * (zfar-znear) + znear;
    const float zt    = tanel_row * len;
    return (float)sqrt((double)len*(double)len + (double)zt*(double)zt);
}

__device__ static inline void hz_unproject_enh(float* lat, float* lon, double range_enh,
                                               float sin_az, float cos_az, double cos_el,
                                               double lat_viewer, double cos_lat_viewer, double lon_viewer)
{
    const float Rearth = 6371000.0;
    double range_en = cos_el * range_enh;
    float e = range_en * sin_az;
    float n = range_en * cos_az;
    *lon = lon_viewer + e / Rearth / M_PI * 180. / cos_lat_viewer;
    *lat = lat_viewer + n / Rearth / M_PI * 180.;
}

__global__ __launch_bounds__(256)
void k_link_cells(const unsigned long long* __restrict__ fb, const float* __restrict__ tanel,
                  const float* __restrict__ sin_az, const float* __restrict__ cos_az, const double* __restrict__ cos_el,
                  float* __restrict__ lat, float* __restrict__ lon,
                  int W, int H, int cell_w, int cell_h, int nx, int ny,
                  float znear, float zfar, double viewer_lat, double cos_viewer_lat, double viewer_lon)
{
    const int c = blockIdx.x*blockDim.x + threadIdx.x;
    if(c >= nx*ny) return;
    const int cy = c / nx, cx = c - cy*nx;
    const int x = cx*cell_w, y = cy*cell_h;
    const int row = H-1-y;
    const float range = hz_range_of(fb[(size_t)row*W + x], tanel[row], znear, zfar);
    float la = __builtin_nanf(""), lo = __builtin_nanf("");
    if(range > 0.0f)
        hz_unproject_enh(&la, &lo, (double)range, sin_az[cx], cos_az[cx], cos_el[cy],
                         viewer_lat, cos_viewer_lat, viewer_lon);
    lat[c] = la; lon[c] = lo;
}

__global__ __launch_bounds__(256)
void k_poi(const unsigned long long* __restrict__ fb, const float* __restrict__ tanel,
           const hz_poi_proj_t* __restrict__ proj, int npois,
           unsigned char* __restrict__ visible, float* __restrict__ label_x, float* __restrict__ label_y,
           int W, int H, int height_out, float znear, float zfar)
{
    const int k = blockIdx.x*blockDim.x + threadIdx.x;
    if(k >= npois) return;
    visible[k] = 0; label_x[k] = 0.f; label_y[k] = 0.f;
    const double cx = proj[k].x, cy = proj[k].y, range_have = proj[k].range;
    if(!(range_have >= 0.0)) return;
    if(range_have < 500.0 || range_have > 100000.0) return;
    int    fuzz_nearest = 0;
    double err_nearest  = 1.7976931348623157e308;
    const int xi = (int)round(cx), yi = (int)round(cy);
    for(int fuzz = -6; fuzz < 6; fuzz++)
    {
        if(cy + (double)fuzz < 0) continue;
        if(cy + (double)fuzz >= height_out) break;
        const int y = yi + fuzz;
        if(y < 0 || y >= H || xi < 0 || xi >= W) continue;
        const int row = H-1-y;
        const float range = hz_range_of(fb[(size_t)row*W + xi], tanel[row], znear, zfar);
        if(range <= 0.0f) continue;
        const double err = fabs(range_have - (double)range);
        if(err < err_nearest) { err_nearest = err; fuzz_nearest = fuzz; }
        else break;
    }
    if(err_nearest < 500.)
    {
        visible[k] = 1;
        label_x[k] = (float)cx;
        label_y[k] = (float)(cy + (float)fuzz_nearest);
    }
}


__global__ __launch_bounds__(256)
void k_polar_fill(const int16_t* __restrict__ mosaic, hz_polar_t* __restrict__ q, int N, hz_xform_t u)
{
    const int i = (int)(blockIdx.x*blockDim.x + threadIdx.x);
    if(i >= N) return;
    const float e = hz_east(&u, (float)i);
    for(int j = (int)blockIdx.y; j < N; j += (int)gridDim.y)
        q[(size_t)j*N + i] = hz_polar_en(&u, e, hz_north(&u, (float)j), (float)mosaic[(size_t)j*N + i]);
}


#include "hz_launch.h"

void hzk_clip(bool wave_items, dim3 grid, dim3 block, hipStream_t stream, const int16_t* mosaic, unsigned long long* fb, mr_queue_t q, hz_params_t p)
{
    if(wave_items) hipLaunchKernelGGL(k_clip<true>, grid, block, 0, stream, mosaic, fb, q, p);
    else hipLaunchKernelGGL(k_clip<false>, grid, block, 0, stream, mosaic, fb, q, p);
}

void hzk_hiz(dim3 grid, dim3 block, hipStream_t stream, const unsigned long long* fb, const unsigned char* touched, int seg_stride, int SW, int H, hz_hiz_t hz, unsigned int nunits)
{
    hipLaunchKernelGGL(k_hiz, grid, block, 0, stream, fb, touched, seg_stride, SW, H, hz, nunits);
}

void hzk_mid(dim3 grid, dim3 block, hipStream_t stream, unsigned long long* fb, const hz_rec_t* midrec, const unsigned int* counters, unsigned int midrec_capacity, hz_params_t p)
{
    hipLaunchKernelGGL(k_mid, grid, block, 0, stream, fb, midrec, counters, midrec_capacity, p);
}

void hzk_march(bool counters, bool hiz, bool vcache, dim3 grid, dim3 block, hipStream_t stream, const int16_t* mosaic, unsigned long long* fb, mr_queue_t q, mr_zones_t zn, hz_params_t p)
{
    const bool shards = p.qshards_log2 != 0;
#ifdef HZ_SELFTEST
    if(counters)
    {
        if(shards) hipLaunchKernelGGL((k_march<true, true, false, true>), grid, block, 0, stream, mosaic, fb, q, zn, p);
        else hipLaunchKernelGGL((k_march<true, true, false, false>), grid, block, 0, stream, mosaic, fb, q, zn, p);
        return;
    }
#endif
    (void)counters;
    #define HZK_MARCH(H, V, S) hipLaunchKernelGGL((k_march<false, H, V, S>), grid, block, 0, stream, mosaic, fb, q, zn, p)
    if(shards)
    {
        if(vcache) { if(hiz) HZK_MARCH(true, true, true); else HZK_MARCH(false, true, true); }
        else       { if(hiz) HZK_MARCH(true, false, true); else HZK_MARCH(false, false, true); }
    }
    else
    {
        if(vcache) { if(hiz) HZK_MARCH(true, true, false); else HZK_MARCH(false, true, false); }
        else       { if(hiz) HZK_MARCH(true, false, false); else HZK_MARCH(false, false, false); }
    }
    #undef HZK_MARCH
}

void hzk_polar_fill(dim3 grid, dim3 block, hipStream_t stream, const int16_t* mosaic, hz_polar_t* q, int N, hz_xform_t u)
{
    hipLaunchKernelGGL(k_polar_fill, grid, block, 0, stream, mosaic, q, N, u);
}

void hzk_resolve(bool clear, dim3 grid, dim3 block, hipStream_t stream, unsigned long long* fb, const float* tanel, unsigned char* bgr, float* ranges, int32_t* index, uint32_t* z24, int SW, int H, float znear, float zfar, unsigned int* qa, unsigned int* qb)
{
    if(clear) hipLaunchKernelGGL(k_resolve<true>, grid, block, 0, stream, fb, tanel, bgr, ranges, index, z24, SW, H, znear, zfar, qa, qb);
    else hipLaunchKernelGGL(k_resolve<false>, grid, block, 0, stream, fb, tanel, bgr, ranges, index, z24, SW, H, znear, zfar, qa, qb);
}

void hzk_resolve4(bool clear, dim3 grid, dim3 block, hipStream_t stream, unsigned long long* fb, const float* tanel, unsigned char* bgr, float* ranges, int32_t* index, uint32_t* z24, int SW, int H, float znear, float zfar, unsigned char* touched, int seg_stride, unsigned int* qa, unsigned int* qb, int yo0, int yo1, int nt)
{
    if(clear) hipLaunchKernelGGL(k_resolve4<true>, grid, block, 0, stream, fb, tanel, bgr, ranges, index, z24, SW, H, znear, zfar, touched, seg_stride, qa, qb, yo0, yo1, nt);
    else hipLaunchKernelGGL(k_resolve4<false>, grid, block, 0, stream, fb, tanel, bgr, ranges, index, z24, SW, H, znear, zfar, touched, seg_stride, qa, qb, yo0, yo1, nt);
}

void hzk_pack_host(bool clear, dim3 grid, dim3 block, hipStream_t stream, unsigned long long* fb, hz_hostpack_t o, int SW, int H, int col_off, unsigned char* touched, int seg_stride, unsigned int* qa, unsigned int* qb)
{
    if(clear) hipLaunchKernelGGL(k_pack_host<true>, grid, block, 0, stream, fb, o, SW, H, col_off, touched, seg_stride, qa, qb);
    else hipLaunchKernelGGL(k_pack_host<false>, grid, block, 0, stream, fb, o, SW, H, col_off, touched, seg_stride, qa, qb);
}

void hzk_tell(hipStream_t stream, hz_tell_t s)
{
    hipLaunchKernelGGL(k_tell, dim3(1), dim3(TELL_THREADS), 0, stream, s);
}

void hzk_pack(bool clear, dim3 grid, dim3 block, hipStream_t stream, unsigned long long* fb, uint32_t* packed, int SW, int H, unsigned int* qa, unsigned int* qb)
{
    if(clear) hipLaunchKernelGGL(k_pack<true>, grid, block, 0, stream, fb, packed, SW, H, qa, qb);
    else hipLaunchKernelGGL(k_pack<false>, grid, block, 0, stream, fb, packed, SW, H, qa, qb);
}

void hzk_resolve_packed(dim3 grid, dim3 block, hipStream_t stream, const uint32_t* packed, int stride, int ncols, const float* tanel, unsigned char* bgr, float* ranges, int out_W, int out_col0, int H, float znear, float zfar)
{
    hipLaunchKernelGGL(k_resolve_packed, grid, block, 0, stream, packed, stride, ncols, tanel, bgr, ranges, out_W, out_col0, H, znear, zfar);
}

void hzk_pack_sparse(bool clear, dim3 grid, dim3 block, hipStream_t stream, unsigned long long* fb, uint32_t* out, int SW, int H, int mask_stride, unsigned char* touched, int seg_stride, unsigned int* qa, unsigned int* qb)
{
    if(clear) hipLaunchKernelGGL(k_pack_sparse<true>, grid, block, 0, stream, fb, out, SW, H, mask_stride, touched, seg_stride, qa, qb);
    else hipLaunchKernelGGL(k_pack_sparse<false>, grid, block, 0, stream, fb, out, SW, H, mask_stride, touched, seg_stride, qa, qb);
}

void hzk_resolve_sparse(dim3 grid, dim3 block, hipStream_t stream, hz_strips_t st, int mask_stride, const float* tanel, unsigned char* bgr, float* ranges, int out_W, int H, float znear, float zfar)
{
    hipLaunchKernelGGL(k_resolve_sparse, grid, block, 0, stream, st, mask_stride, tanel, bgr, ranges, out_W, H, znear, zfar);
}

void hzk_scatter(dim3 grid, dim3 block, hipStream_t stream, const int16_t* mosaic, unsigned long long* fb, mr_queue_t q, hz_params_t p)
{
    hipLaunchKernelGGL(k_scatter, grid, block, 0, stream, mosaic, fb, q, p);
}

void hzk_big(dim3 grid, dim3 block, hipStream_t stream, unsigned long long* fb, const hz_bigrec_t* bigrec, const hz_bigitem_t* bigitem, const unsigned int* big_counters, unsigned int bigrec_capacity, unsigned int bigitem_capacity, hz_params_t p, const unsigned int* tile_state, unsigned int* report)
{
    if(p.qshards_log2 != 0) hipLaunchKernelGGL(k_big<true>, grid, block, 0, stream, fb, bigrec, bigitem, big_counters, bigrec_capacity, bigitem_capacity, p, tile_state, report);
    else hipLaunchKernelGGL(k_big<false>, grid, block, 0, stream, fb, bigrec, bigitem, big_counters, bigrec_capacity, bigitem_capacity, p, tile_state, report);
}

void hzk_shade_tex(dim3 grid, dim3 block, hipStream_t stream, const unsigned long long* fb, const int16_t* mosaic, const uint32_t* texels, hz_texparams_t tp, unsigned char* bgr, hz_params_t p)
{
    hipLaunchKernelGGL(k_shade_tex, grid, block, 0, stream, fb, mosaic, texels, tp, bgr, p);
}

void hzk_tile_bin(dim3 grid, dim3 block, hipStream_t stream, const hz_bigrec_t* bigrec, const hz_bigitem_t* bigitem, const unsigned int* big_counters, unsigned int bigrec_capacity, tl_bins_t tb, hz_params_t p)
{
    hipLaunchKernelGGL(k_tile_bin, grid, block, 0, stream, bigrec, bigitem, big_counters, bigrec_capacity, tb, p);
}

void hzk_tile_raster(dim3 grid, dim3 block, hipStream_t stream, unsigned long long* fb, const hz_bigrec_t* bigrec, tl_bins_t tb, hz_params_t p)
{
    hipLaunchKernelGGL(k_tile_raster, grid, block, 0, stream, fb, bigrec, tb, p);
}

void hzk_ingest(dim3 grid, dim3 block, hipStream_t stream, const unsigned char* const* tiles, int16_t* mosaic, int N, int ntx, int nty, int cpd, int oc_x, int oc_y)
{
    hipLaunchKernelGGL(k_ingest, grid, block, 0, stream, tiles, mosaic, N, ntx, nty, cpd, oc_x, oc_y);
}

void hzk_link_cells(dim3 grid, dim3 block, hipStream_t stream, const unsigned long long* fb, const float* tanel, const float* sin_az, const float* cos_az, const double* cos_el, float* lat, float* lon, int W, int H, int cell_w, int cell_h, int nx, int ny, float znear, float zfar, double viewer_lat, double cos_viewer_lat, double viewer_lon)
{
    hipLaunchKernelGGL(k_link_cells, grid, block, 0, stream, fb, tanel, sin_az, cos_az, cos_el, lat, lon, W, H, cell_w, cell_h, nx, ny, znear, zfar, viewer_lat, cos_viewer_lat, viewer_lon);
}

void hzk_poi(dim3 grid, dim3 block, hipStream_t stream, const unsigned long long* fb, const float* tanel, const hz_poi_proj_t* proj, int npois, unsigned char* visible, float* label_x, float* label_y, int W, int H, int height_out, float znear, float zfar)
{
    hipLaunchKernelGGL(k_poi, grid, block, 0, stream, fb, tanel, proj, npois, visible, label_x, label_y, W, H, height_out, znear, zfar);
}

#ifdef HZ_SELFTEST
#include "hz_dev.h"
#include "hz_selftest.h"
#include "hz_selftest_impl.h"
#endif
```

### horizonator_amd/csrc/hz_launch.h

```cpp
#pragma once

#include <hip/hip_runtime_api.h>

#include "hz_types.h"

void hzk_clip(bool wave_items, dim3 grid, dim3 block, hipStream_t stream, const int16_t* mosaic, unsigned long long* fb, mr_queue_t q, hz_params_t p);
void hzk_hiz(dim3 grid, dim3 block, hipStream_t stream, const unsigned long long* fb, const unsigned char* touched, int seg_stride, int SW, int H, hz_hiz_t hz, unsigned int nunits);
void hzk_mid(dim3 grid, dim3 block, hipStream_t stream, unsigned long long* fb, const hz_rec_t* midrec, const unsigned int* counters, unsigned int midrec_capacity, hz_params_t p);
void hzk_march(bool counters, bool hiz, bool vcache, dim3 grid, dim3 block, hipStream_t stream, const int16_t* mosaic, unsigned long long* fb, mr_queue_t q, mr_zones_t zn, hz_params_t p);
void hzk_resolve(bool clear, dim3 grid, dim3 block, hipStream_t stream, unsigned long long* fb, const float* tanel, unsigned char* bgr, float* ranges, int32_t* index, uint32_t* z24, int SW, int H, float znear, float zfar, unsigned int* qa, unsigned int* qb);
void hzk_resolve4(bool clear, dim3 grid, dim3 block, hipStream_t stream, unsigned long long* fb, const float* tanel, unsigned char* bgr, float* ranges, int32_t* index, uint32_t* z24, int SW, int H, float znear, float zfar, unsigned char* touched, int seg_stride, unsigned int* qa, unsigned int* qb, int yo0, int yo1, int nt);
void hzk_pack_host(bool clear, dim3 grid, dim3 block, hipStream_t stream, unsigned long long* fb, hz_hostpack_t o, int SW, int H, int col_off, unsigned char* touched, int seg_stride, unsigned int* qa, unsigned int* qb);
void hzk_tell(hipStream_t stream, hz_tell_t s);
void hzk_pack(bool clear, dim3 grid, dim3 block, hipStream_t stream, unsigned long long* fb, uint32_t* packed, int SW, int H, unsigned int* qa, unsigned int* qb);
void hzk_resolve_packed(dim3 grid, dim3 block, hipStream_t stream, const uint32_t* packed, int stride, int ncols, const float* tanel, unsigned char* bgr, float* ranges, int out_W, int out_col0, int H, float znear, float zfar);
void hzk_pack_sparse(bool clear, dim3 grid, dim3 block, hipStream_t stream, unsigned long long* fb, uint32_t* out, int SW, int H, int mask_stride, unsigned char* touched, int seg_stride, unsigned int* qa, unsigned int* qb);
void hzk_resolve_sparse(dim3 grid, dim3 block, hipStream_t stream, hz_strips_t st, int mask_stride, const float* tanel, unsigned char* bgr, float* ranges, int out_W, int H, float znear, float zfar);
void hzk_scatter(dim3 grid, dim3 block, hipStream_t stream, const int16_t* mosaic, unsigned long long* fb, mr_queue_t q, hz_params_t p);
void hzk_big(dim3 grid, dim3 block, hipStream_t stream, unsigned long long* fb, const hz_bigrec_t* bigrec, const hz_bigitem_t* bigitem, const unsigned int* big_counters, unsigned int bigrec_capacity, unsigned int bigitem_capacity, hz_params_t p, const unsigned int* tile_state, unsigned int* report);
void hzk_shade_tex(dim3 grid, dim3 block, hipStream_t stream, const unsigned long long* fb, const int16_t* mosaic, const uint32_t* texels, hz_texparams_t tp, unsigned char* bgr, hz_params_t p);
void hzk_tile_bin(dim3 grid, dim3 block, hipStream_t stream, const hz_bigrec_t* bigrec, const hz_bigitem_t* bigitem, const unsigned int* big_counters, unsigned int bigrec_capacity, tl_bins_t tb, hz_params_t p);
void hzk_tile_raster(dim3 grid, dim3 block, hipStream_t stream, unsigned long long* fb, const hz_bigrec_t* bigrec, tl_bins_t tb, hz_params_t p);
void hzk_ingest(dim3 grid, dim3 block, hipStream_t stream, const unsigned char* const* tiles, int16_t* mosaic, int N, int ntx, int nty, int cpd, int oc_x, int oc_y);
void hzk_link_cells(dim3 grid, dim3 block, hipStream_t stream, const unsigned long long* fb, const float* tanel, const float* sin_az, const float* cos_az, const double* cos_el, float* lat, float* lon, int W, int H, int cell_w, int cell_h, int nx, int ny, float znear, float zfar, double viewer_lat, double cos_viewer_lat, double viewer_lon);
void hzk_poi(dim3 grid, dim3 block, hipStream_t stream, const unsigned long long* fb, const float* tanel, const hz_poi_proj_t* proj, int npois, unsigned char* visible, float* label_x, float* label_y, int W, int H, int height_out, float znear, float zfar);
void hzk_polar_fill(dim3 grid, dim3 block, hipStream_t stream, const int16_t* mosaic, hz_polar_t* q, int N, hz_xform_t u);
```

### horizonator_amd/csrc/hz_plan.cpp

```cpp
#include "hz_dev.h"
#include "hz_fast.h"

mr_zones_t hz_make_zones(const hz_params_t& p, bool near_first)
{
    const float ppr = p.halfW * p.u.az_ndc_per_rad;
    const int   ncr = p.N-1;
    const float vj  = p.u.viewer_cell_j;
    const int r2  = (int)(ppr/16.f) + 1;
    const int r4  = (int)(ppr/4.f) + 1;
    const int r16 = (int)(ppr/1.f) + 1;
    auto clampi = [&](float x) { int v = (int)floorf(x); if(v < 0) v = 0; if(v > ncr) v = ncr; return v; };
    mr_zones_t z;
    z.row0[0] = 0;
    z.row0[1] = clampi(vj - (float)r16);
    z.row0[2] = clampi(vj - (float)r4);
    z.row0[3] = clampi(vj - (float)r2);
    z.row0[4] = clampi(vj + (float)r2 + 1.f);
    z.row0[5] = clampi(vj + (float)r4 + 1.f);
    z.row0[6] = clampi(vj + (float)r16 + 1.f);
    z.row0[7] = ncr;
    int far_rows = 64*p.SW/p.W;
    if(far_rows < 16) far_rows = 16;
    if(far_rows > 32) far_rows = 32;
    const int z16 = 6*p.SW < p.W ? 8 : 16;
    const float cells_to_zfar = sqrtf(p.far_dd)/(p.u.deg_per_cell*111194.9f);
    const int z4 = cells_to_zfar <= 0.25f*ppr ? 2 : 4;
    int rows[MR_NZONES] = { far_rows, z16, z4, 2, z4, z16, far_rows };
    if(p.SW == p.W)
    {
        long waves = 0;
        for(int k=0; k<MR_NZONES; k++) waves += (z.row0[k+1] - z.row0[k] + rows[k]-1)/rows[k];
        waves *= (p.N-1 + MR_COLS-1)/MR_COLS;
        if(waves < 32768) { rows[0] = rows[6] = rows[0] < 16 ? rows[0] : 16; rows[1] = rows[5] = rows[1] < 8 ? rows[1] : 8; rows[2] = rows[4] = 2; }
    }
    const int order_far_first [MR_NZONES] = { 0, 6, 1, 5, 2, 4, 3 };
    const int order_near_first[MR_NZONES] = { 3, 2, 4, 1, 5, 0, 6 };
    z.near_first = near_first ? 1 : 0;
    const int* order = near_first ? order_near_first : order_far_first;
    int seg = 0;
    for(int o=0; o<MR_NZONES; o++)
    {
        const int k = order[o];
        z.rows[k] = rows[k];
        z.seg0[k] = seg;
        const int n = z.row0[k+1] - z.row0[k];
        z.nseg[k] = (n + rows[k]-1)/rows[k];
        seg += z.nseg[k];
    }
    z.total = seg;
    return z;
}

hz_params_t hz_make_params(const hz_dev_t* d, const hz_view_t* v)
{
    hz_params_t p;
    memset(&p, 0, sizeof(p));
    p.u.viewer_cell_i  = v->viewer_cell_i;
    p.u.viewer_cell_j  = v->viewer_cell_j;
    p.u.viewer_z       = v->viewer_z;
    p.u.cos_viewer_lat = v->cos_viewer_lat;
    p.u.deg_per_cell   = v->deg_per_cell;
    p.u.aspect         = v->aspect;
    p.u.znear          = v->znear;
    p.u.zfar           = v->zfar;
    p.u.znear_color    = v->znear_color;
    p.u.zfar_color     = v->zfar_color;
    hz_frame_from_az(v->az_deg0, v->az_deg1, &p.u.az_center, &p.u.az_ndc_per_rad);
    p.halfW = (float)d->W * 0.5f;
    p.halfH = (float)d->H * 0.5f;
    p.N = d->N; p.W = d->W; p.H = d->H;
    p.col0 = d->col0; p.col1 = d->col1; p.SW = d->col1 - d->col0;
    p.touched = d->d_touched[d->fbi]; p.seg_stride = d->seg_stride;
    p.inline_max = (p.SW == p.W) ? HZ_INLINE_MAX_PIX : 16;
    p.far_dd = (v->zfar*1.001f)*(v->zfar*1.001f);
    {
        const float e0 = hz_abs(hz_east(&p.u, 0.f)),  e1 = hz_abs(hz_east(&p.u, (float)(p.N-1)));
        const float n0 = hz_abs(hz_north(&p.u, 0.f)), n1 = hz_abs(hz_north(&p.u, (float)(p.N-1)));
        const float em = e0 > e1 ? e0 : e1, nm = n0 > n1 ? n0 : n1;
        p.far_strips = !(nm*nm + em*em <= p.far_dd);
    }
    p.big_min    = HZ_INLINE_MAX_PIX;
    p.z_guard = 1.0f/500.0f + (float)(d->W > d->H ? d->W : d->H) * (1.0f/4194304.0f);
    p.z_hide_k = 1.03f * p.z_guard * 16777215.f;
    p.quad_max_dx = d->W >= 64 && d->W <= 65535 && d->H <= 65535 ? 256*(d->W/16 - 1) : 0;
#ifdef HZ_EXPERIMENTS
    p.exp_fb[HZ_WHO_MARCH] = d->exp.exp_fb_march; p.exp_fb[HZ_WHO_BIG] = d->exp.exp_fb_big;
    p.debug   = d->exp.march_debug;
#endif
    p.pretest_march = 0;
    p.fast_ok = hzf_draw_ok(&p.u) && d->env.fast_math;
    return p;
}


static void ray_sincos(double a, double* s, double* c)
{
    static thread_local double ka[4] = { 1e300, 1e300, 1e300, 1e300 }, ks[4], kc[4];
    static thread_local int turn = 0;
    for(int k=0; k<4; k++) if(ka[k] == a) { *s = ks[k]; *c = kc[k]; return; }
    const int k = turn++ & 3;
    ka[k] = a; ks[k] = sin(a); kc[k] = cos(a);
    *s = ks[k]; *c = kc[k];
}

static bool wedge_band_extent(double a0, double a1, double n_lo, double n_hi, double* lo, double* hi)
{
    const double inf = 1e300;
    double e_lo = inf, e_hi = -inf;
    auto add = [&](double e) { if(e < e_lo) e_lo = e; if(e > e_hi) e_hi = e; };
    if(n_lo <= 0.0 && 0.0 <= n_hi) add(0.0);
    const double rays[2] = { a0, a1 };
    for(int r=0; r<2; r++)
    {
        double s, c;
        ray_sincos(rays[r], &s, &c);
        if(fabs(c) < 1e-12)
        {
            if(n_lo <= 0.0 && 0.0 <= n_hi) add(s > 0 ? inf : -inf);
            continue;
        }
        const double bounds[2] = { n_lo, n_hi };
        for(int b=0; b<2; b++)
        {
            const double t = bounds[b]/c;
            if(t >= 0.0) add(t*s);
        }
    }
    if(e_lo > e_hi) return false;
    auto contains = [&](double dir) { double x = fmod(dir - a0, 2.0*M_PI); if(x < 0) x += 2.0*M_PI; return x <= a1 - a0; };
    if(contains( 0.5*M_PI)) e_hi =  inf;
    if(contains(-0.5*M_PI)) e_lo = -inf;
    *lo = e_lo; *hi = e_hi;
    return true;
}

static bool strips_behind_columns(const hz_params_t& p, double a0, double a1, int jbeg, int jend, int nsx, int* x0, int* x1)
{
    const double m_per_cell_n = (double)HZ_REARTH_PI * (double)p.u.deg_per_cell / 180.0;
    const double m_per_cell_e = m_per_cell_n * (double)p.u.cos_viewer_lat;
    const double n_lo = ((double)(jbeg-1) - (double)p.u.viewer_cell_j) * m_per_cell_n;
    const double n_hi = ((double)(jend+1) - (double)p.u.viewer_cell_j) * m_per_cell_n;
    double lo = 0, hi = 0;
    bool any = false;
    const int parts = (a1 - a0 > M_PI) ? 2 : 1;
    for(int k=0; k<parts; k++)
    {
        const double b0 = a0 + (a1 - a0)*k/parts, b1 = a0 + (a1 - a0)*(k+1)/parts;
        double l, h;
        if(!wedge_band_extent(b0, b1, n_lo, n_hi, &l, &h)) continue;
        if(!any) { lo = l; hi = h; any = true; }
        else { if(l < lo) lo = l; if(h > hi) hi = h; }
    }
    if(!any) return false;
    double i_lo = lo/m_per_cell_e + (double)p.u.viewer_cell_i - 2.0, i_hi = hi/m_per_cell_e + (double)p.u.viewer_cell_i + 2.0;
    if(!(i_lo > -1e9)) i_lo = -1e9;
    if(!(i_hi <  1e9)) i_hi =  1e9;
    int a = (int)ceil(i_lo/(double)MR_COLS) - 1, b = (int)floor(i_hi/(double)MR_COLS);
    if(a < 0) a = 0;
    if(b > nsx-1) b = nsx-1;
    if(a > b) return false;
    *x0 = a; *x1 = b;
    return true;
}

bool hz_azimuths_of_columns(const hz_params_t& p, double* a0, double* a1)
{
    const double k = (double)p.u.az_ndc_per_rad, c = (double)p.u.az_center, hw = (double)p.halfW;
    const double lo = c + (((double)p.col0 - 4.0)/hw - 1.0)/k, hi = c + (((double)p.col1 + 4.0)/hw - 1.0)/k;
    if(!(hi - lo < 2.0*M_PI - 1e-3) || !(hi > lo)) return false;
    *a0 = lo; *a1 = hi;
    return true;
}

void hz_list_rounds(const hz_params_t& p, const mr_zones_t& zn, double a0, double a1, bool one_round,
                    std::vector<uint32_t>* first, std::vector<uint32_t>& second, bool every_strip)
{
    const int nsx = (p.N-1 + MR_COLS-1)/MR_COLS;
    if(first) first->clear();
    second.clear();
    const double m_per_cell_n = (double)HZ_REARTH_PI * (double)p.u.deg_per_cell / 180.0;
    const double m_per_cell_e = m_per_cell_n * (double)p.u.cos_viewer_lat;
    const int parts = (a1 - a0 > M_PI) ? 2 : 1;
    double ray[3][2];
    for(int k=0; k<=parts; k++) { const double a = a0 + (a1 - a0)*k/parts; ray[k][0] = sin(a); ray[k][1] = cos(a); }
    for(int seg=0; seg<zn.total; seg++)
    {
        int jbeg, jend;
        mr_segment_rows(zn, seg, &jbeg, &jend);
        int x0 = 0, x1 = nsx-1;
        if(!every_strip && !strips_behind_columns(p, a0, a1, jbeg, jend, nsx, &x0, &x1)) continue;
        const bool near_rows = jbeg < p.near_j1 && jend > p.near_j0;
        const double n_lo = ((double)(jbeg-1) - (double)p.u.viewer_cell_j) * m_per_cell_n;
        const double n_hi = ((double)(jend+1) - (double)p.u.viewer_cell_j) * m_per_cell_n;
        auto reaches = [&](int sx) -> bool
        {
            const double e_lo = ((double)(sx*MR_COLS - 2) - (double)p.u.viewer_cell_i) * m_per_cell_e;
            const double e_hi = ((double)(sx*MR_COLS + MR_COLS + 2) - (double)p.u.viewer_cell_i) * m_per_cell_e;
            if(e_lo <= 0.0 && 0.0 <= e_hi && n_lo <= 0.0 && 0.0 <= n_hi) return true;
            for(int k=0; k<parts; k++)
            {
                const double c[4][2] = { { e_lo, n_lo }, { e_hi, n_lo }, { e_lo, n_hi }, { e_hi, n_hi } };
                bool before_first = true, beyond_second = true;
                for(int q=0; q<4; q++)
                {
                    if(!(ray[k][0]*c[q][1] - ray[k][1]*c[q][0] > 0.0))   before_first = false;
                    if(!(ray[k+1][0]*c[q][1] - ray[k+1][1]*c[q][0] < 0.0)) beyond_second = false;
                }
                if(!before_first && !beyond_second) return true;
            }
            return false;
        };
        if(!every_strip && parts == 1)
        {
            while(x0 <= x1 && !reaches(x0)) x0++;
            while(x1 > x0 && !reaches(x1)) x1--;
        }
        for(int sx=x0; sx<=x1; sx++)
        {
            if(!every_strip && parts == 2 && !reaches(sx)) continue;
            const bool near = !one_round && near_rows && sx >= p.near_x0 && sx <= p.near_x1;
            if(near) { if(first) first->push_back(MR_ITEM(seg, sx)); }
            else second.push_back(MR_ITEM(seg, sx));
        }
    }
}

void hz_list_items(const hz_params_t& p, const mr_zones_t& zn, double a0, double a1, std::vector<uint32_t>& out, bool every_strip)
{
    if(p.pass == 1) { std::vector<uint32_t> rest; hz_list_rounds(p, zn, a0, a1, false, &out, rest, every_strip); }
    else hz_list_rounds(p, zn, a0, a1, p.pass == 0, NULL, out, every_strip);
}

int hz_plan_rounds(const hz_dev_t* d, const hz_view_t* view, hz_params_t& p)
{
    const int nsx = (p.N-1 + MR_COLS-1)/MR_COLS;
    int near_cells = d->env.near_cells;
    if(near_cells < 0)
    {
        const float ppr = p.halfW * p.u.az_ndc_per_rad;
        near_cells = (int)(ppr / HZ_NEAR_PX + 0.5f);
        if(near_cells < 16) near_cells = 16;
        if(near_cells > HZ_NEAR_CELLS_WIDE) near_cells = HZ_NEAR_CELLS_WIDE;
        if(ppr/(float)HZ_NEAR_CELLS_MAX >= HZ_HIZ_MIN_PX && (d->env.adapt == 2 || (d->env.adapt == 1 && d->adapt.long_reach))) near_cells = HZ_NEAR_CELLS_MAX;
    }
    p.near_x0 = (int)floorf((p.u.viewer_cell_i - (float)near_cells)/(float)MR_COLS);
    p.near_x1 = (int)floorf((p.u.viewer_cell_i + (float)near_cells)/(float)MR_COLS);
    if(p.near_x0 < 0) p.near_x0 = 0;
    if(p.near_x1 > nsx-1) p.near_x1 = nsx-1;
    p.near_j0 = (int)floorf(p.u.viewer_cell_j - (float)near_cells);
    p.near_j1 = (int)ceilf (p.u.viewer_cell_j + (float)near_cells);
    const float cells_to_zfar = view->zfar / (p.u.deg_per_cell * 111194.9f);
    const bool want_two = d->env.rounds > 0 ? d->env.rounds == 2
                             : ((double)p.W*(double)p.H >= HZ_TWO_ROUNDS_MIN_PIX && cells_to_zfar >= 3.0f*(float)near_cells);
    return want_two && near_cells > 0 && p.near_x1 >= p.near_x0 ? 2 : 1;
}
```

### horizonator_amd/csrc/hz_selftest_impl.h

```cpp
#pragma once

__device__ static inline unsigned long long hz_mix64(unsigned long long x)
{
    x += 0x9E3779B97F4A7C15ull;
    x = (x ^ (x >> 30)) * 0xBF58476D1CE4E5B9ull;
    x = (x ^ (x >> 27)) * 0x94D049BB133111EBull;
    return x ^ (x >> 31);
}
__device__ static inline float hz_seeded_float(unsigned long long r, int elo, int ehi)
{
    const uint32_t mant = (uint32_t)r & 0x7FFFFFu, sign = (uint32_t)(r >> 23) & 1u;
    const uint32_t ex = (uint32_t)elo + (uint32_t)((r >> 24) % (unsigned long long)(ehi - elo + 1));
    return __uint_as_float((sign << 31) | (ex << 23) | mant);
}

__global__ __launch_bounds__(256)
void k_check_fastmath(int what, unsigned long long seed, unsigned long long n, unsigned long long* mismatches, float* first_bad)
{
    unsigned long long bad = 0;
    for(unsigned long long k = (unsigned long long)blockIdx.x*blockDim.x + threadIdx.x; k < n; k += (unsigned long long)gridDim.x*blockDim.x)
    {
        float a = 0.f, b = 0.f, want = 0.f, got = 0.f;
        bool in_range = true;
        if(what == 0)
        {
            b = __uint_as_float((uint32_t)k);
            in_range = hz_abs(b) >= 2.16840434e-19f && hz_abs(b) <= 4.61168602e18f;
            if(in_range) { want = 1.0f / b; got = hzf_rcp(b); }
        }
        else if(what == 1)
        {
            b = __uint_as_float((uint32_t)k);
            in_range = b >= 1.26217745e-29f && b <= 3.40282347e38f;
            if(in_range) { want = __builtin_sqrtf(b); got = hzf_sqrt(b); }
        }
        else if(what == 2)
        {
            const unsigned long long r1 = hz_mix64(seed + 2*k), r2 = hz_mix64(seed + 2*k + 1);
            a = hz_seeded_float(r1, 127-60, 127+60);
            b = hz_seeded_float(r2, 127-31, 127+31);
            if((r2 >> 61) == 1) { const float t = hz_abs(a); a = hz_min(t, 1.0f); b = hz_max(t, 1.0f); }
            if((r2 >> 61) == 2) a = __uint_as_float((__float_as_uint(a) & 0xFF800000u) | (__float_as_uint(b) & 0x7FFFFFu));
            if((r1 >> 60) == 0) a = 0.0f;
            want = a / b; got = hzf_div(a, b);
        }
        else if(what == 4)
        {
            const double dd = (double)(k + 1);
            const double r = hz_rcp_f64(dd);
            const double rel = __builtin_fabs(__builtin_fma(dd, r, -1.0));
            a = (float)dd; b = (float)rel; want = 0.f; got = rel < 8.8817841970012523e-16 ? 0.f : 1.f;
        }
        else if(what == 5)
        {
            const unsigned long long r1 = hz_mix64(seed + 2*k), r2 = hz_mix64(seed + 2*k + 1);
            const int32_t d = (int32_t)(((r2 >> 8) & 0x7FFFFFFFull) >> (r2 & 31)) | 1;
            int64_t n = (int64_t)(r1 >> 9) >> ((r1 >> 3) & 63);
            if(r1 & 1) n = -n;
            if((r1 & 6) == 2) n = (n / d)*(int64_t)d + (int64_t)((r2 >> 40) % 3) - 1;
            int64_t q = n / d;
            if((n % d) != 0 && n < 0) q--;
            const int32_t f = hz_floor_div(n, d, hz_rcp_f64((double)d));
            a = (float)n; b = (float)d;
            const bool ok = (q > 1073741824ll) ? f >= 1073741824 : (q < -1073741824ll) ? f <= -1073741824 : (int64_t)f == q;
            want = 0.f; got = ok ? 0.f : 1.f;
        }
        else if(what == 6)
        {
            float two_pi = HZ_TWO_PI;
            asm volatile("" : "+v"(two_pi));
            b = two_pi;
            a = __uint_as_float((uint32_t)k);
            const float aa = hz_abs(a);
            in_range = __float_as_uint(a) == 0u || (aa >= 7.88860905e-31f && aa <= 1073741824.0f);
            if(in_range) { want = a / b; got = hzf_div_by_two_pi(a, hzf_refined_rcp(two_pi)); }
        }
        else if(what == 7)
        {
            a = __uint_as_float((uint32_t)k);
            in_range = __float_as_uint(a) == 0u || (a >= 2.16840434e-19f && a <= 4.61168602e18f);
            if(in_range) { want = hz_min(a, 1.0f) / hz_max(a, 1.0f); got = hzf_fold_to_unit(a); }
        }
        else if(what == 8 || what == 9)
        {
            const unsigned long long r1 = hz_mix64(seed + 2*k), r2 = hz_mix64(seed + 2*k + 1);
            a = hz_seeded_float(r1, 127-30, 127+29);
            b = hz_seeded_float(r2, 127-30, 127+29);
            if((r1 >> 60) == 0 && what == 9) a = 0.0f;
            if((r1 >> 60) == 1) a = __uint_as_float((__float_as_uint(a) & 0x80000000u) | (__float_as_uint(b) & 0x7FFFFFFFu));
            if((r1 >> 60) == 2) a = __uint_as_float(__float_as_uint(a) & 0xFFFFFF00u);
            if((r2 >> 60) == 2) b = __uint_as_float(__float_as_uint(b) & 0xFFFFFF00u);
            if(what == 9) b = hz_abs(b) * (((r2 >> 59) & 1) ? 1.41421354f : 1.0f);
            want = hz_atan2(a, b);
            got  = what == 9 ? hzf_atan2<true>(a, b) : hzf_atan2<false>(a, b);
        }
        else
        {
            b = __uint_as_float((uint32_t)seed);
            a = __uint_as_float((uint32_t)k);
            const float aa = hz_abs(a);
            in_range = __float_as_uint(a) == 0u || (aa >= 7.88860905e-31f && aa <= 1.15292150e18f);
            if(in_range) { want = a / b; got = hzf_div_by(a, b, hzf_refined_rcp(b)); }
        }
        if(in_range && __float_as_uint(want) != __float_as_uint(got))
        {
            if(bad == 0 && atomicAdd(mismatches + 1, 1ull) == 0) { first_bad[0] = a; first_bad[1] = b; first_bad[2] = want; first_bad[3] = got; }
            bad++;
        }
    }
    if(bad) atomicAdd(mismatches, bad);
}

extern "C" int hz_hip_check_fastmath(int device, int what, unsigned long long seed, unsigned long long n,
                                     unsigned long long* mismatches, float* first_bad)
{
    hz_device_guard device_guard_(device);
    if(!device_guard_.ok) return -1;
    if(what < 0 || what > 9) { snprintf(g_last_error, sizeof(g_last_error), "hz_hip_check_fastmath: what = %d", what); return -1; }
    if(what == 0 || what == 1 || what == 3 || what == 6 || what == 7) n = 1ull << 32;
    if(what == 4) n = (1ull << 31) - 1;
    unsigned long long* d_bad = NULL; float* d_first = NULL;
    HZ_CHECK(hipMalloc(&d_bad, 2*sizeof(unsigned long long)));
    HZ_CHECK(hipMalloc(&d_first, 4*sizeof(float)));
    HZ_CHECK(hipMemset(d_bad, 0, 2*sizeof(unsigned long long)));
    HZ_CHECK(hipMemset(d_first, 0, 4*sizeof(float)));
    hipLaunchKernelGGL(k_check_fastmath, dim3(256*32), dim3(256), 0, 0, what, seed, n, d_bad, d_first);
    HZ_CHECK(hipGetLastError());
    unsigned long long h[2] = {0, 0};
    HZ_CHECK(hipMemcpy(h, d_bad, sizeof(h), hipMemcpyDeviceToHost));
    if(first_bad) HZ_CHECK(hipMemcpy(first_bad, d_first, 4*sizeof(float), hipMemcpyDeviceToHost));
    *mismatches = h[0];
    (void)hipFree(d_bad); (void)hipFree(d_first);
    return 0;
}


__global__ __launch_bounds__(256)
void k_check_hidden(unsigned long long seed, unsigned long long n, int W, int H, unsigned long long* out)
{
    const float z_guard = 1.0f/500.0f + (float)(W > H ? W : H) * (1.0f/4194304.0f);
    const float kk = 1.03f * z_guard * 16777215.f;
    unsigned long long tested = 0, hidden = 0, frags = 0, bad = 0, margin = ~0ull;
    for(unsigned long long t = (unsigned long long)blockIdx.x*blockDim.x + threadIdx.x; t < n; t += (unsigned long long)gridDim.x*blockDim.x)
    {
        const unsigned long long r0 = hz_mix64(seed + 4*t), r1 = hz_mix64(seed + 4*t + 1), r2 = hz_mix64(seed + 4*t + 2), r3 = hz_mix64(seed + 4*t + 3);
        auto unit = [](unsigned long long r, int shift) { return (float)((r >> shift) & 0xFFFFFFull) * (1.0f/16777216.0f); };
        const int family = (int)(r0 & 3);
        float bx = unit(r0, 8) * (float)W, by = unit(r0, 32) * (float)H;
        if(((r0 >> 2) & 7) == 0) bx = (float)W - 4.0f*unit(r1, 0);
        if(((r0 >> 5) & 7) == 0) by = (float)H - 4.0f*unit(r1, 24);
        float x[3], y[3], z[3];
        const float ext = family == 3 ? 16.0f*unit(r3, 40) : family == 0 ? 2.5f : 4.0f;
        x[0] = bx; y[0] = by;
        x[1] = bx + (unit(r1, 8) - 0.5f)*ext;  y[1] = by + (unit(r1, 36) - 0.5f)*ext;
        x[2] = bx + (unit(r2, 0) - 0.5f)*ext;  y[2] = by + (unit(r2, 24) - 0.5f)*ext;
        if(family == 1)
        {
            const float tt = unit(r2, 0)*1.5f - 0.25f, off = __builtin_ldexpf(1.0f, -1 - (int)((r2 >> 40) % 14)) * ((r2 >> 63) ? 1.0f : -1.0f);
            const float dx = x[1] - x[0], dy = y[1] - y[0], len = hz_sqrt(dx*dx + dy*dy) + 1e-6f;
            x[2] = x[0] + tt*dx - off*dy/len; y[2] = y[0] + tt*dy + off*dx/len;
        }
        const float zb = 0.02f + 0.96f*unit(r3, 0);
        const float dz = (family == 2 ? 6e-3f : 1e-3f) * __builtin_ldexpf(1.0f, -(int)((r3 >> 24) % 18));
        z[0] = zb; z[1] = zb + (unit(r3, 30) - 0.5f)*dz; z[2] = zb + (unit(r2, 40) - 0.5f)*dz;
        hz_wvert_t v[3];
        bool inside = true;
        for(int k=0; k<3; k++)
        {
            v[k].xn = 0.f; v[k].wx = x[k]; v[k].wy = y[k]; v[k].zw = z[k]; v[k].red = 0.25f*(float)k; v[k].cmask = 0;
            inside = inside && x[k] >= 0.f && x[k] <= (float)W && y[k] >= 0.f && y[k] <= (float)H && z[k] >= 0.f && z[k] <= 1.f;
            v[k].xs = (int32_t)hz_roundeven((x[k] - 0.5f)*256.f);
            v[k].ys = (int32_t)hz_roundeven((y[k] - 0.5f)*256.f);
        }
        if(!inside) continue;
        hz_box_t box;
        if(!hz_tri_cull_window(&box, &v[0], &v[1], &v[2], 0, W-1, 0, H-1))
        {
            const hz_wvert_t tmp = v[1]; v[1] = v[2]; v[2] = tmp;
            if(!hz_tri_cull_window(&box, &v[0], &v[1], &v[2], 0, W-1, 0, H-1)) continue;
        }
        tested++;
        if(!hz_tri_hidden(&v[0], &v[1], &v[2], kk, 0u)) continue;
        uint32_t lo = 0, hi = HZ_Z24_MAX;
        if(hz_tri_hidden(&v[0], &v[1], &v[2], kk, hi)) lo = hi;
        while(hi - lo > 1u)
        {
            const uint32_t mid = lo + (hi - lo)/2u;
            if(hz_tri_hidden(&v[0], &v[1], &v[2], kk, mid)) lo = mid; else hi = mid;
        }
        hidden++;
        hz_tri_t tri;
        hz_tri_planes(&tri, &v[0], &v[1], &v[2]);
        for(int py = box.py0; py <= box.py1; py++)
            for(int px = box.px0; px <= box.px1; px++)
            {
                if(!hz_tri_covers(&tri, px, py)) continue;
                uint32_t zi, r8;
                if(!hz_tri_fragment(&tri, px, py, &zi, &r8)) continue;
                frags++;
                if(zi <= lo) bad++;
                const unsigned long long m = (unsigned long long)((long long)zi - (long long)lo + (1ll << 32));
                if(m < margin) margin = m;
            }
    }
    atomicAdd(&out[0], tested); atomicAdd(&out[1], hidden); atomicAdd(&out[2], frags); atomicAdd(&out[3], bad);
    atomicMin(&out[4], margin);
}

__global__ __launch_bounds__(64)
void k_check_cull(unsigned long long seed, unsigned long long ncases, int W, int H, int col0, int col1, unsigned long long* out)
{
    hz_params_t p;
    memset(&p, 0, sizeof(p));
    p.halfW = (float)W*0.5f; p.halfH = (float)H*0.5f; p.W = W; p.H = H; p.col0 = col0; p.col1 = col1; p.SW = col1 - col0;
    p.quad_max_dx = W >= 64 && W <= 65535 && H <= 65535 ? 256*(W/16 - 1) : 0;
    const int lane = threadIdx.x;
    const bool has_cell = lane < MR_COLS;
    unsigned long long cases = 0, shortway = 0, cells = 0, bad = 0, kept = 0;
    for(unsigned long long t = blockIdx.x; t < ncases; t += gridDim.x)
    {
        const unsigned long long rc = hz_mix64(seed + 977*t);
        auto unit = [](unsigned long long r, int shift) { return (float)((r >> shift) & 0xFFFFFFull) * (1.0f/16777216.0f); };
        const int kind = (int)(rc & 7);
        float step = 2.0f/(float)W * (0.1f + 8.0f*unit(rc, 8));
        if(kind == 5) step = -step;
        const float jump = kind <= 2 ? 2.0f/16.0f * (0.97f + 0.06f*unit(rc, 44)) : 0.0f;
        const int   jump_lane = (int)((rc >> 3) & 63);
        const float x_first = kind == 1 ? -1.0f : kind == 2 ? 1.0f - 63.0f*step - jump : -1.0f + (2.0f - 64.0f*hz_abs(step) - jump)*unit(rc, 32);
        const float y_base  = ((rc >> 56) & 3) == 0 ? 1.0f - 4.0f/(float)H*unit(rc, 40) : -1.0f + 2.0f*unit(rc, 40);
        hz_vertex_t vt[2];
        for(int row=0; row<2; row++)
        {
            const unsigned long long r = hz_mix64(seed + 977*t + 131*(unsigned long long)(row + 1) + 7*(unsigned long long)lane);
            float xn = x_first + (float)lane*step + (lane > jump_lane ? jump : 0.0f) + (unit(r, 0) - 0.5f)*hz_abs(step)*0.6f;
            float yn = y_base + (row ? 1 : 0)*(2.0f/(float)H)*(0.2f + 4.0f*unit(rc, 16)) + (unit(r, 24) - 0.5f)*(2.0f/(float)H);
            float zn = -1.0f + 2.0f*unit(r, 40);
            if(kind == 4 && ((r >> 60) & 3) == 0)
                xn = ((float)(int)(unit(r, 8)*(float)W) + (((r >> 59) & 1) ? 0.5f : 0.0f))/p.halfW - 1.0f;
            if(kind == 6 && lane >= 32) xn -= 1.9f*unit(rc, 20);
            if(kind == 7 && ((r >> 58) & 15) == 0)
            {
                const float edge[4] = { 1.0f, -1.0f, 1.00000012f, -1.00000012f };
                if((r >> 62) & 1) xn = edge[(r >> 56) & 3]; else if((r >> 63) & 1) yn = edge[(r >> 56) & 3]; else zn = edge[(r >> 56) & 3];
            }
            vt[row].x = xn; vt[row].y = yn; vt[row].z = zn; vt[row].red = 0.5f;
        }
        mr_rowstate_t st[2];
        hz_wvert_t wv[2];
        bool simple[2];
        for(int row=0; row<2; row++)
        {
            bool in_volume, in_guard;
            wv[row] = mr_window(vt[row], p, &in_volume, &in_guard);
            simple[row] = __all(in_guard && in_volume);
            if(!simple[row]) mr_window_flags(wv[row], vt[row], in_guard);
            st[row] = mr_rowstate_of(wv[row], p);
        }
        cases++;
        bool keep0 = false, keep1 = false;
        if(!(simple[0] && simple[1] && mr_simple_cull(st[0], st[1], has_cell, p, &keep0, &keep1))) continue;
        shortway++;
        hz_wvert_t v00 = {}, v01 = {}, v10 = {}, v11 = {};
        v00.xn = st[0].xn; v00.xs = st[0].xs; v00.ys = st[0].ys; v00.cmask = st[0].cmask;
        v01.xn = st[1].xn; v01.xs = st[1].xs; v01.ys = st[1].ys; v01.cmask = st[1].cmask;
        v10.xn = mr_from_east(st[0].xn); v10.xs = mr_from_east(st[0].xs); v10.ys = mr_from_east(st[0].ys); v10.cmask = (uint32_t)mr_from_east((int32_t)st[0].cmask);
        v11.xn = mr_from_east(st[1].xn); v11.xs = mr_from_east(st[1].xs); v11.ys = mr_from_east(st[1].ys); v11.cmask = (uint32_t)mr_from_east((int32_t)st[1].cmask);
        if(has_cell)
        {
            hz_box_t box;
            const bool want0 = hz_tri_cull(&box, &v00, &v11, &v01, p.col0, p.col1-1, 0, p.H-1) == HZ_TRI_DRAW;
            const bool want1 = hz_tri_cull(&box, &v00, &v10, &v11, p.col0, p.col1-1, 0, p.H-1) == HZ_TRI_DRAW;
            cells++;
            if(want0 != keep0) bad++;
            if(want1 != keep1) bad++;
            kept += (keep0 ? 1 : 0) + (keep1 ? 1 : 0);
        }
    }
    atomicAdd(&out[0], lane == 0 ? cases : 0ull); atomicAdd(&out[1], lane == 0 ? shortway : 0ull);
    atomicAdd(&out[2], cells); atomicAdd(&out[3], bad); atomicAdd(&out[4], kept);
}

__global__ __launch_bounds__(256)
void k_check_rect(unsigned long long seed, unsigned long long ncases, int W, int H, unsigned long long* out)
{
    unsigned long long cases = 0, numbers = 0, pixels = 0, bad = 0, nans = 0;
    for(unsigned long long t = (unsigned long long)blockIdx.x*blockDim.x + threadIdx.x; t < ncases; t += (unsigned long long)gridDim.x*blockDim.x)
    {
        const unsigned long long r0 = hz_mix64(seed + 3*t), r1 = hz_mix64(seed + 3*t + 1), r2 = hz_mix64(seed + 3*t + 2);
        auto unit = [](unsigned long long r, int shift) { return (float)((r >> shift) & 0xFFFFFFull) * (1.0f/16777216.0f); };
        auto slope = [&](unsigned long long r) -> float
        {
            const int kind = (int)(r & 15);
            if(kind == 0) return 0.0f;
            if(kind == 1) return (r >> 4) & 1 ? __builtin_inff() : -__builtin_inff();
            if(kind == 2) return __builtin_nanf("");
            if(kind == 3) return ((r >> 4) & 1 ? 1.0f : -1.0f) * 3.0e38f * unit(r, 8);
            const float mag = exp2f(-40.0f + 60.0f*unit(r, 8));
            return ((r >> 4) & 1) ? mag : -mag;
        };
        hz_tri_t tri;
        memset(&tri, 0, sizeof(tri));
        tri.dzdx = slope(r0); tri.dzdy = slope(r1);
        tri.z_org = ((r2 & 7) == 0) ? -3.0f + 7.0f*unit(r2, 8) : unit(r2, 8);
        if((r2 & 63) == 1) tri.z_org = __builtin_inff();
        const int bw = 1 + (int)((r2 >> 32) % 48u), bh = 1 + (int)((r2 >> 40) % 48u);
        const int x0 = (int)((r0 >> 32) % (unsigned long long)(W - bw + 1)), y0 = (int)((r1 >> 32) % (unsigned long long)(H - bh + 1));
        if((r2 >> 48) & 1) tri.z_org = 0.5f - tri.dzdx*(float)(x0 + bw/2) - tri.dzdy*(float)(y0 + bh/2);
        uint32_t qmin = 0;
        const bool ok = hiz_rect_min_depth(tri, x0, x0 + bw - 1, y0, y0 + bh - 1, &qmin);
        uint32_t m = 0xFFFFFFFFu;
        bool nan_inside = false;
        for(int py = y0; py < y0 + bh; py++)
            for(int px = x0; px < x0 + bw; px++)
            {
                float z = __builtin_fmaf(tri.dzdy, (float)py, __builtin_fmaf(tri.dzdx, (float)px, tri.z_org));
                if(!(z == z)) { nan_inside = true; continue; }
                z = hz_min(hz_max(z, 0.f), 1.f);
                const uint32_t q = (uint32_t)hz_roundeven(z * 16777215.f);
                uint32_t zi, r8;
                const int drawn = hz_tri_fragment(&tri, px, py, &zi, &r8);
                if(drawn && zi != q) bad++;
                m = m < q ? m : q;
            }
        cases++; pixels += (unsigned long long)bw*bh;
        if(nan_inside) nans++;
        if(ok) { numbers++; if(nan_inside || m != qmin) bad++; }
    }
    atomicAdd(&out[0], cases); atomicAdd(&out[1], numbers); atomicAdd(&out[2], pixels); atomicAdd(&out[3], bad); atomicAdd(&out[4], nans);
}

extern "C" int hz_hip_check_exactness(int device, int what, unsigned long long seed, unsigned long long n,
                                      int W, int H, int col0, int col1, unsigned long long* out)
{
    hz_device_guard device_guard_(device);
    if(!device_guard_.ok) return -1;
    if(what < 0 || what > 2 || W < 1 || H < 1 || col0 < 0 || col1 > W || col0 >= col1 || (what == 2 && (W < 48 || H < 48)))
    {
        snprintf(g_last_error, sizeof(g_last_error), "hz_hip_check_exactness: bad arguments");
        return -1;
    }
    unsigned long long* d_out = NULL;
    HZ_CHECK(hipMalloc(&d_out, 5*sizeof(unsigned long long)));
    const unsigned long long init[5] = { 0, 0, 0, 0, what == 0 ? ~0ull : 0ull };
    HZ_CHECK(hipMemcpy(d_out, init, sizeof(init), hipMemcpyHostToDevice));
    if(what == 0)      hipLaunchKernelGGL(k_check_hidden, dim3(256*32), dim3(256), 0, 0, seed, n, W, H, d_out);
    else if(what == 1) hipLaunchKernelGGL(k_check_cull, dim3(256*64), dim3(64), 0, 0, seed, n, W, H, col0, col1, d_out);
    else               hipLaunchKernelGGL(k_check_rect, dim3(256*16), dim3(256), 0, 0, seed, n, W, H, d_out);
    HZ_CHECK(hipGetLastError());
    HZ_CHECK(hipMemcpy(out, d_out, 5*sizeof(unsigned long long), hipMemcpyDeviceToHost));
    (void)hipFree(d_out);
    return 0;
}

extern "C" int hz_hip_debug_bigqueue(hz_dev_t* d, int set, unsigned int* counters, int max_rec, int32_t* recs)
{
    HZ_ON_DEVICE(d);
    if(hz_hip_sync(d) != 0) return -1;
    const int k = (set ? HZ_NFB : 0) + d->fbi;
    std::vector<unsigned int> all(HZ_NCOUNTERS);
    HZ_CHECK(hipMemcpy(all.data(), d->d_big_counters_s[k], HZ_NCOUNTERS*sizeof(unsigned int), hipMemcpyDeviceToHost));
    unsigned int per_shard[HZ_QSHARDS], longest = 0;
    const int sl = d->last_qshards_log2;
    if(d->fb_consumed) { for(int c=0; c<6; c++) counters[c] = all[HZ_CNT_LAST + c]; for(int s=0; s<HZ_QSHARDS; s++) per_shard[s] = 0; }
    else
    {
        counters[0] = counters[1] = 0; counters[2] = 0; counters[3] = 0; counters[5] = 0;
        for(int s=0; s<HZ_QSHARDS; s++)
        {
            const unsigned int* c = all.data() + HZ_QSHARD0 + s*HZ_QSHARD_STRIDE;
            per_shard[s] = c[0] < HZ_QSHARD_ROOM(d->bigrec_capacity, sl) ? c[0] : HZ_QSHARD_ROOM(d->bigrec_capacity, sl);
            counters[0] += c[0]; counters[1] += c[1]; if(c[2]) counters[2] = c[2];
            counters[3] += c[4]; if(c[5]) counters[5] = c[5];
            if(per_shard[s] > longest) longest = per_shard[s];
        }
        counters[4] = all[4];
    }
    counters[2] = ~counters[2]; counters[5] = ~counters[5];
    if(longest == 0 || recs == NULL || max_rec <= 0) return 0;
    const size_t slots = (size_t)((longest + HZ_QBLOCK-1)/HZ_QBLOCK*HZ_QBLOCK) << sl;
    hz_bigrec_t* h = (hz_bigrec_t*)malloc(slots*sizeof(hz_bigrec_t));
    if(!h) return -1;
    HZ_CHECK(hipMemcpy(h, d->d_bigrec_s[k], slots*sizeof(hz_bigrec_t), hipMemcpyDeviceToHost));
    int n = 0;
    for(size_t g=0; g<slots && n<max_rec; g++)
    {
        const size_t block = g >> HZ_QBLOCK_LOG2;
        if((((block >> sl) << HZ_QBLOCK_LOG2) | (g & (HZ_QBLOCK-1))) >= per_shard[block & (((size_t)1 << sl) - 1)]) continue;
        int32_t* o = recs + (size_t)n*10;
        o[0] = h[g].r.px0; o[1] = h[g].r.py0; o[2] = h[g].r.bw; o[3] = h[g].bh;
        for(int m=0; m<3; m++) { o[4+m] = h[g].r.e.dx[m]; o[7+m] = -h[g].r.e.ndy[m]; }
        n++;
    }
    free(h);
    return 0;
}

extern "C" long hz_hip_debug_worklist(int N, int W, int H, const hz_view_t* view, int col0, int col1, int round,
                                      int32_t* out, size_t capacity_items)
{
    hz_dev_t* d = (hz_dev_t*)calloc(1, sizeof(*d));
    if(!d) return -1;
    d->env = hz_options_from_env();
    d->N = N; d->W = W; d->H = H; d->col0 = col0; d->col1 = col1;
    d->seg_stride = (W + HZ_SEG-1)/HZ_SEG;
    hz_params_t p = hz_make_params(d, view);
    (void)hz_plan_rounds(d, view, p);
    const mr_zones_t zn = hz_make_zones(p, (round & 3) != 0);
    free(d);
    p.pass = round & 3;
    double a0 = 0, a1 = 0;
    const bool every_strip = (round & 256) != 0;
    if(!every_strip && !hz_azimuths_of_columns(p, &a0, &a1)) return -1;
    std::vector<uint32_t> items;
    hz_list_items(p, zn, a0, a1, items, every_strip);
    for(size_t k=0; k<items.size() && k<capacity_items; k++)
    {
        int jbeg, jend;
        mr_segment_rows(zn, (int)(items[k] >> MR_ITEM_SX_BITS), &jbeg, &jend);
        out[3*k] = (int32_t)(items[k] & ((1u << MR_ITEM_SX_BITS) - 1u)); out[3*k+1] = jbeg; out[3*k+2] = jend;
    }
    return (long)items.size();
}

extern "C" int hz_hip_debug_wave_timing(hz_dev_t* d, const hz_view_t* view, unsigned long long* out, size_t capacity_words, unsigned int* grid)
{
    HZ_ON_DEVICE(d);
    HZ_CHECK(hz_sync_all(d));
    unsigned long long* d_cycles = NULL;
    HZ_CHECK(hipMalloc(&d_cycles, capacity_words*sizeof(unsigned long long)));
    HZ_CHECK(hipMemset(d_cycles, 0, capacity_words*sizeof(unsigned long long)));
    d->wave_timing.d_cycles = d_cycles; d->wave_timing.capacity = capacity_words;
    d->wave_timing.grid_x = d->wave_timing.grid_y = 0;
    int rc = hz_draw_impl(d, view);
    d->wave_timing.d_cycles = NULL; d->wave_timing.capacity = 0;
    if(rc == 0 && hz_sync_all(d) != hipSuccess) rc = -1;
    grid[0] = d->wave_timing.grid_x; grid[1] = d->wave_timing.grid_y;
    if(rc == 0 && hipMemcpy(out, d_cycles, (size_t)grid[0]*grid[1]*4*sizeof(unsigned long long), hipMemcpyDeviceToHost) != hipSuccess) rc = -1;
    (void)hipFree(d_cycles);
    return rc;
}
```

### horizonator_amd/csrc/hz_types.h

```cpp
#pragma once

#include <stddef.h>
#include <stdint.h>

#include "hz_raster.h"
#include "hz_tex.h"
#include "hz_scatter.h"


struct hz_hiz_t { uint32_t* l1; uint32_t* l2; int w1, w2; };

#define HZ_WHO_MARCH 0
#define HZ_WHO_BIG   1
#define HZ_WHO_OTHER 2

struct hz_params_t
{
    hz_xform_t u;
    float halfW, halfH;
    int   N;
    int   W, H;
    int   col0, col1;
    int   SW;
    unsigned long long* wave_cycles;
    unsigned int inline_max;
    unsigned int big_min;
    float far_dd;
    int   far_strips;
    const uint32_t* worklist;
    int   cull_strips;
    int   pass;
    int   near_x0, near_x1;
    int   near_j0, near_j1;
    int   early_z;
    int   pretest_march;
    int   qshards_log2;
#ifdef HZ_EXPERIMENTS
    int   exp_fb[2];
#endif
    const hz_polar_t* vcache;
    const uint32_t* hiz;
    float z_guard;
    float z_hide_k;
    int   fast_ok;
    int   quad_max_dx;
#ifdef HZ_EXPERIMENTS
    int   debug;
#endif
    unsigned char* touched;
    int   seg_stride;
};
#define HZ_SEG_LOG2 8
#define HZ_SEG      (1 << HZ_SEG_LOG2)

struct hz_rec_t
{
    hz_edges_t e;
    float    z_org, dzdx, dzdy, r_org, drdx, drdy;
    int32_t  px0, py0, bw;
    float    inv_bw;
    uint32_t prim;
};
struct hz_bigrec_t { hz_rec_t r; int32_t bh; };

struct hz_bigitem_t { uint32_t rec; uint32_t chunk; };

struct mr_queue_t
{
    hz_bigrec_t*  bigrec;
    hz_bigitem_t* bigitem;
    hz_rec_t*     midrec;
    uint32_t*     clip;
    unsigned int* counters;
    unsigned int  bigrec_capacity, bigitem_capacity, midrec_capacity, clip_capacity;
};

#define HZ_QSHARDS_LOG2  4
#define HZ_QSHARDS       (1 << HZ_QSHARDS_LOG2)
#define HZ_QBLOCK_LOG2   4
#define HZ_QBLOCK        (1 << HZ_QBLOCK_LOG2)
#define HZ_QSHARD_ROOM(capacity, sl) ((((capacity) >> ((sl) + HZ_QBLOCK_LOG2))) << HZ_QBLOCK_LOG2)
#define HZ_QSLOT(l, s, sl) (((((((uint32_t)(l)) >> HZ_QBLOCK_LOG2) << (sl)) + (uint32_t)(s)) << HZ_QBLOCK_LOG2) | (((uint32_t)(l)) & (HZ_QBLOCK-1)))
#define HZ_QSHARD_STRIDE 32
#define HZ_QSHARD0       16
#define HZ_NCOUNTERS (HZ_QSHARD0 + HZ_QSHARDS*HZ_QSHARD_STRIDE)
#define HZ_CNT_LAST  8
#ifndef HZ_NFB
#define HZ_NFB 3
#endif
#define HZ_STAGE_SLOTS 32
#define HZ_STAGE_BYTES ((size_t)4 << 20)
#define HZ_COPY_STREAMS 2
#define HZ_HOST_BANDS  4
#define HZ_INLINE_MAX_PIX  64


#define MR_COLS   63
#define HZ_NEAR_CELLS_WIDE 384
#define HZ_NEAR_CELLS_MAX  512

#define MR_NZONES 7
struct mr_zones_t
{
    int row0[MR_NZONES+1];
    int rows[MR_NZONES];
    int seg0[MR_NZONES];
    int nseg[MR_NZONES];
    int total;
    int near_first;
};

HZ_HD void mr_segment_rows(const mr_zones_t& zn, int seg, int* jbeg, int* jend)
{
    int zone = 0;
    #pragma unroll
    for(int z=1; z<MR_NZONES; z++)
        if(seg >= zn.seg0[z] && seg < zn.seg0[z] + zn.nseg[z]) zone = z;
    int sseg = seg - zn.seg0[zone];
    if(zn.near_first && zone < MR_NZONES/2) sseg = zn.nseg[zone]-1 - sseg;
    const int jb = zn.row0[zone] + sseg*zn.rows[zone];
    const int je = jb + zn.rows[zone];
    *jbeg = jb;
    *jend = je < zn.row0[zone+1] ? je : zn.row0[zone+1];
}

#define MR_ITEM_SX_BITS 12
#define MR_ITEM(seg, sx) (((uint32_t)(seg) << MR_ITEM_SX_BITS) | (uint32_t)(sx))


#define TL_W 64
#define TL_H 64

#define TL_LIST 2048
#define TL_BATCH 64
#define TL_ROW_MIN 24
#define TL_UNITS_PER_TILE 4

struct tl_bins_t
{
    unsigned int* cursor;
    unsigned int* pairs;
    unsigned int* state;
    unsigned int* busy;
    unsigned int  units_cap;
    int           tiles_x, tiles_y;
    unsigned int  list_cap;
};

#define HIZ1_W_LOG2 3
#define HIZ1_H_LOG2 2
#define HIZ2_W_LOG2 5
#define HIZ2_H_LOG2 4
#define HIZ_UNIT_ROWS 16

HZ_HD size_t hiz_w1(int SW) { return (size_t)((SW + (1 << HIZ1_W_LOG2) - 1) >> HIZ1_W_LOG2); }
HZ_HD size_t hiz_w2(int SW) { return (size_t)((SW + (1 << HIZ2_W_LOG2) - 1) >> HIZ2_W_LOG2); }
HZ_HD size_t hiz_h1(int H)  { return (size_t)((H  + (1 << HIZ1_H_LOG2) - 1) >> HIZ1_H_LOG2); }
HZ_HD size_t hiz_h2(int H)  { return (size_t)((H  + (1 << HIZ2_H_LOG2) - 1) >> HIZ2_H_LOG2); }
HZ_HD size_t hiz_words(int W, int H) { return hiz_w1(W)*hiz_h1(H) + hiz_w2(W)*hiz_h2(H); }

#define SC_CX 64
#define SC_CY 4
#define SC_VX (SC_CX+1)
#define SC_VY (SC_CY+1)
#define SC_THREADS (SC_CX*SC_CY)

#define TX_SUB   4
#define TX_CHUNK (64*TX_SUB)

struct hz_hostpack_t
{
    uint32_t*     out;
    unsigned int* cursor;
    unsigned int  capacity;
    unsigned int  chunk_words;
    uint32_t      flags;
    unsigned int* present;
};
#define HP_NONE 0xFFFFFFFFu

struct hz_tell_t
{
    const unsigned int* cursor;
    const unsigned int* present;
    unsigned int*       h_info;
    unsigned int*       h_present;
    unsigned int        capacity;
    unsigned int        npresent;
    unsigned int        epoch;
};


#define SP_WAVES  4
#define SP_STEPS  8
#define SP_MAXIT  256

#define HZ_MAX_STRIPS 16
struct hz_strips_t
{
    const uint32_t* in[HZ_MAX_STRIPS];
    int ncols[HZ_MAX_STRIPS], col0[HZ_MAX_STRIPS];
};
```

### include/hz_selftest.h

```cpp
#pragma once

#include "hz_hip.h"

#ifdef __cplusplus
extern "C" {
#endif

int  hz_hip_check_fastmath(int device, int what, unsigned long long seed, unsigned long long n,
                           unsigned long long* mismatches, float* first_bad);

int  hz_hip_check_exactness(int device, int what, unsigned long long seed, unsigned long long n,
                            int W, int H, int col0, int col1, unsigned long long* out);

int  hz_hip_debug_bigqueue(hz_dev_t* d, int set, unsigned int* counters, int max_rec, int32_t* recs);

long hz_hip_debug_worklist(int N, int W, int H, const hz_view_t* view, int col0, int col1, int round,
                           int32_t* out, size_t capacity_items);

int  hz_hip_debug_wave_timing(hz_dev_t* d, const hz_view_t* view, unsigned long long* out, size_t capacity_words, unsigned int* grid);

#ifdef __cplusplus
}
#endif
```

Measured before the change: 82480.

## Compute per-strip conservative facts to skip far tests, atan folding, and wide-cell checks

Adds a per-strip analysis at the start of the march kernel that bounds the strip's extent and uses the mosaic's elevation range, now computed at upload and ingest, to prove three facts. These are: no rows are far, the elevation atan2 argument never exceeds 1, and cells are narrow and away from the azimuth seam. When a fact holds, the kernel skips the per-row far-distance wave votes, the atan fold and reciprocal, and the wide-quad min/max check in the simple cull. The cost is a small per-strip prologue, an extra min/max reduction kernel at ingest (and a host loop on upload), and correctness that rests on the conservative bounds.

After: 82840 (median of 6 runs). Within noise of the previous version (+0.4%).

```diff
diff --git a/horizonator_amd/_lib.py b/horizonator_amd/_lib.py
--- a/horizonator_amd/_lib.py
+++ b/horizonator_amd/_lib.py
@@ -204,6 +204,7 @@
         sig("hz_hip_debug_bigqueue", i, vp, i, vp, i, vp)
         sig("hz_hip_debug_wave_timing", i, vp, P(View), vp, C.c_size_t, vp)
         sig("hz_hip_debug_worklist", C.c_long, i, i, i, P(View), i, i, i, vp, C.c_size_t)
+        sig("hz_hip_debug_strip_facts", i, i, i, i, P(View), vp, i, i, i, i, i, i, vp)
     return lib
 
 
@@ -231,7 +232,7 @@
     "hz_hip_read_depth", "hz_hip_link_cells", "hz_hip_poi_visibility", "hz_hip_sync", "hz_hip_last_times", "hz_hip_stream", "hz_hip_wait_outputs", "hz_hip_wait_for", "hz_hip_last_plan", "hz_hip_last_queue_counts", "hz_hip_last_error",
 ]
 SELFTEST_SYMBOLS = ["hz_hip_check_fastmath", "hz_hip_check_exactness", "hz_hip_debug_bigqueue", "hz_hip_debug_wave_timing",
-                    "hz_hip_debug_worklist"]
+                    "hz_hip_debug_worklist", "hz_hip_debug_strip_facts"]
 
 
 def load_demgen():
diff --git a/horizonator_amd/csrc/hz_context.cpp b/horizonator_amd/csrc/hz_context.cpp
--- a/horizonator_amd/csrc/hz_context.cpp
+++ b/horizonator_amd/csrc/hz_context.cpp
@@ -178,6 +178,7 @@
     HZ_CHECK(hipEventCreateWithFlags(&d->ev_readers, hipEventDisableTiming));
     HZ_CHECK(hipEventCreateWithFlags(&d->ev_tanel,   hipEventDisableTiming));
     HZ_CHECK(hipMalloc(&d->d_mosaic, (size_t)d->N*d->N*sizeof(int16_t)));
+    d->z_lo = -32768; d->z_hi = 32767;
     sw.lap("streams, events, mosaic");
     d->seg_stride = (d->W + HZ_SEG-1) / HZ_SEG;
     for(int i=0; i<HZ_NFB; i++)
@@ -267,8 +268,12 @@
 {
     HZ_ON_DEVICE(d);
     HZ_CHECK(hz_sync_all(d));
+    d->z_lo = -32768; d->z_hi = 32767;
     HZ_CHECK(hipMemcpyAsync(d->d_mosaic, mosaic, (size_t)d->N*d->N*sizeof(int16_t), hipMemcpyHostToDevice, d->stream));
+    int lo = 32767, hi = -32768;
+    for(size_t k = 0, n = (size_t)d->N*d->N; k < n; k++) { const int z = mosaic[k]; lo = z < lo ? z : lo; hi = z > hi ? z : hi; }
     HZ_CHECK(hipStreamSynchronize(d->stream));
+    d->z_lo = lo; d->z_hi = hi;
     d->adapt.have_view = 0;
     d->vc.state = 0;
     return 0;
diff --git a/horizonator_amd/csrc/hz_dev.h b/horizonator_amd/csrc/hz_dev.h
--- a/horizonator_amd/csrc/hz_dev.h
+++ b/horizonator_amd/csrc/hz_dev.h
@@ -95,6 +95,7 @@
     hipStream_t stream, rstream;
     hipEvent_t  ev_drawn, ev_free[HZ_NFB], ev_readers, ev_tanel;
     int16_t*            d_mosaic;
+    int                 z_lo, z_hi;
     unsigned long long* d_fbs[HZ_NFB];
     size_t              fb_used[HZ_NFB];
     int                 fbi;
diff --git a/horizonator_amd/csrc/hz_fast.h b/horizonator_amd/csrc/hz_fast.h
--- a/horizonator_amd/csrc/hz_fast.h
+++ b/horizonator_amd/csrc/hz_fast.h
@@ -57,8 +57,9 @@
     return c;
 }
 
+#define HZF_BRANCH() asm volatile("")
 template<bool XPOS>
-__device__ static inline float hzf_atan2_r(float y, float x, float rcp)
+__device__ static inline float hzf_atan2_r(float y, float x, float rcp, bool unfolded = false)
 {
     const bool  flip = XPOS ? false : (0.f >= x);
     const float ax   = hz_abs(x);
@@ -66,7 +67,9 @@
     const float sot  = s * rcp;
     const float tn   = (ax == hz_abs(y)) ? 1.0f : hz_abs(sot);
 
-    const float u  = hzf_fold_to_unit(tn);
+    float u = tn;
+    bool  folds = false;
+    if(!unfolded) { HZF_BRANCH(); folds = 1.0f < tn; u = folds ? hzf_rcp(tn) : tn; }
     const float u2 = u*u;
     const float u3 = u2*u;
     const float u5 = u3*u2;
@@ -77,26 +80,27 @@
     p = p + u7*-0.1173503194786851f;
     p = p + u9*0.0536813784310406f;
     p = p + (u9*-0.0121323213173444f)*u2;
-    const float a   = (1.0f < tn) ? ((p*-2.0f + HZ_HALF_PI) + p) : p;
+    float a = p;
+    if(!unfolded) { a = folds ? ((p*-2.0f + HZ_HALF_PI) + p) : p; }
     const float arc = flip ? (HZ_HALF_PI + a) : a;
     const uint32_t sign = ((uint32_t)__float_as_int(y) | (uint32_t)__float_as_int(rcp)) & 0x80000000u;
     return __int_as_float((int)((uint32_t)__float_as_int(arc) | sign));
 }
 template<bool XPOS>
-__device__ static inline float hzf_atan2(float y, float x)
+__device__ static inline float hzf_atan2(float y, float x, bool unfolded = false)
 {
     const float t = (XPOS ? false : (0.f >= x)) ? y : hz_abs(x);
-    return hzf_atan2_r<XPOS>(y, x, hzf_rcp(t));
+    return hzf_atan2_r<XPOS>(y, x, hzf_rcp(t), unfolded);
 }
 
-__device__ static inline hz_polar_t hzf_polar_en_r(const hz_xform_t* u, float e, float n, float fz, float rcp_az)
+__device__ static inline hz_polar_t hzf_polar_en_r(const hz_xform_t* u, float e, float n, float fz, float rcp_az, bool el_unfolded = false)
 {
     hz_polar_t q;
     const float h = fz - u->viewer_z;
     const float nn = n*n, ee = e*e;
     q.d_ne  = hzf_sqrt(nn + ee);
     q.az    = hzf_atan2_r<false>(e, n, rcp_az);
-    q.el    = hzf_atan2<true>(h, q.d_ne);
+    q.el    = hzf_atan2<true>(h, q.d_ne, el_unfolded);
     q.d_enh = hzf_sqrt(h*h + nn + ee);
     return q;
 }
@@ -120,9 +124,9 @@
 {
     return hzf_finish(u, c, hzf_polar_en(u, e, n, fz));
 }
-__device__ static inline hz_vertex_t hzf_transform_en_r(const hz_xform_t* u, const hzf_const_t* c, float e, float n, float fz, float rcp_az)
+__device__ static inline hz_vertex_t hzf_transform_en_r(const hz_xform_t* u, const hzf_const_t* c, float e, float n, float fz, float rcp_az, bool el_unfolded = false)
 {
-    return hzf_finish(u, c, hzf_polar_en_r(u, e, n, fz, rcp_az));
+    return hzf_finish(u, c, hzf_polar_en_r(u, e, n, fz, rcp_az, el_unfolded));
 }
 
 #endif
diff --git a/horizonator_amd/csrc/hz_ingest.cpp b/horizonator_amd/csrc/hz_ingest.cpp
--- a/horizonator_amd/csrc/hz_ingest.cpp
+++ b/horizonator_amd/csrc/hz_ingest.cpp
@@ -63,6 +63,18 @@
         hzk_ingest(grid, dim3(256), d->stream, (const unsigned char* const*)d_ptrs, d->d_mosaic, d->N, ntx, nty, cpd, oc_x, oc_y);
         if(hipGetLastError() != hipSuccess) break;
         if(hipStreamSynchronize(d->stream) != hipSuccess) break;
+        d->z_lo = -32768; d->z_hi = 32767;
+        {
+            const int preset[2] = { 32767, -32768 };
+            int range[2] = { 0, 0 };
+            int* d_range = (int*)d_ptrs;
+            if(hipMemcpyAsync(d_range, preset, sizeof(preset), hipMemcpyHostToDevice, d->stream) != hipSuccess) break;
+            hzk_mosaic_range(dim3(1024), dim3(256), d->stream, (const int16_t*)d->d_mosaic, (size_t)d->N*d->N, d_range);
+            if(hipGetLastError() != hipSuccess) break;
+            if(hipMemcpyAsync(range, d_range, sizeof(range), hipMemcpyDeviceToHost, d->stream) != hipSuccess) break;
+            if(hipStreamSynchronize(d->stream) != hipSuccess) break;
+            if(range[0] <= range[1]) { d->z_lo = range[0]; d->z_hi = range[1]; }
+        }
         d->adapt.have_view = 0;
         d->vc.state = 0;
         rc = 0;
diff --git a/horizonator_amd/csrc/hz_k_march.h b/horizonator_amd/csrc/hz_k_march.h
--- a/horizonator_amd/csrc/hz_k_march.h
+++ b/horizonator_amd/csrc/hz_k_march.h
@@ -152,7 +152,7 @@
     return now;
 }
 
-__device__ static inline bool mr_simple_cull(const mr_rowstate_t& prev, const mr_rowstate_t& now, bool has_cell,
+__device__ static inline bool mr_simple_cull(const mr_rowstate_t& prev, const mr_rowstate_t& now, bool has_cell, bool narrow,
                                              const hz_params_t& p, bool* keep0, bool* keep1)
 {
     const int32_t d01x = (int32_t)((uint32_t)now.xs - (uint32_t)prev.xs);
@@ -160,8 +160,12 @@
     const int32_t d11x = (int32_t)((uint32_t)d01x + (uint32_t)now.h_dx);
     const int32_t d11y = (int32_t)((uint32_t)d01y + (uint32_t)now.h_dy);
     const int32_t d10x = prev.h_dx, d10y = prev.h_dy;
-    const int32_t lo = hz_imin(hz_imin(d01x, d11x), d10x), hi = hz_imax(hz_imax(d01x, d11x), d10x);
-    if(__any(has_cell && !(lo > -p.quad_max_dx && hi < p.quad_max_dx))) return false;
+    if(!narrow)
+    {
+        HZF_BRANCH();
+        const int32_t lo = hz_imin(hz_imin(d01x, d11x), d10x), hi = hz_imax(hz_imax(d01x, d11x), d10x);
+        if(__any(has_cell && !(lo > -p.quad_max_dx && hi < p.quad_max_dx))) return false;
+    }
     const int64_t area0 = (int64_t)d11x*(int64_t)d01y - (int64_t)d01x*(int64_t)d11y;
     const int64_t area1 = (int64_t)d10x*(int64_t)d11y - (int64_t)d11x*(int64_t)d10y;
     const uint32_t c0 = mr_pk_min(now.h_c, prev.c),                 f0 = mr_pk_max(now.h_f1, prev.f1);
@@ -404,6 +408,31 @@
     mr_distribute(r, npix, lane, fb, p);
 }
 
+__device__ static inline uint32_t mr_strip_facts(const hz_params_t& p, float e, float n_tab, int jbeg, int jend, bool vcache)
+{
+    const int nrows = jend - jbeg;
+    const float e_a = __builtin_bit_cast(float, __builtin_amdgcn_readlane(__builtin_bit_cast(int, e), 0));
+    const float e_b = __builtin_bit_cast(float, __builtin_amdgcn_readlane(__builtin_bit_cast(int, e), 63));
+    const float n_a = __builtin_bit_cast(float, __builtin_amdgcn_readlane(__builtin_bit_cast(int, n_tab), 0));
+    const float n_b = nrows < 64 ? __builtin_bit_cast(float, __builtin_amdgcn_readlane(__builtin_bit_cast(int, n_tab), nrows))
+                                 : hz_north(&p.u, (float)jend);
+    const hz_strip_ext_t x = hz_strip_extent(n_a, n_b, e_a, e_b);
+    uint32_t facts = 0;
+    if(hz_strip_no_far_rows(&x, p.far_dd)) facts |= HZ_STRIP_NO_FAR_ROWS;
+    if(!vcache && hz_strip_el_unfolded(&x, p.z_lo - p.u.viewer_z, p.z_hi - p.u.viewer_z)) facts |= HZ_STRIP_EL_UNFOLDED;
+    const float cell_n = hz_strip_cell_n(&p.u);
+    if(hz_strip_narrow_cells(&x, cell_n*hz_abs(p.u.cos_viewer_lat), cell_n, p.halfW*hz_abs(p.u.az_ndc_per_rad), p.quad_max_dx >> 8))
+    {
+        const int lane = threadIdx.x;
+        const int c = hz_strip_corner((lane & 1) ? e_b : e_a, (lane & 2) ? n_b : n_a, p.seam_e, p.seam_n);
+        int all4 = 7, any4 = 0;
+        #pragma unroll
+        for(int k=0; k<4; k++) { const int ck = __builtin_amdgcn_readlane(c, k); all4 &= ck; any4 |= ck; }
+        if(hz_strip_off_seam(all4, any4)) facts |= HZ_STRIP_NARROW_CELLS;
+    }
+    return facts;
+}
+
 #ifdef MR_WAVES_PER_EU
 #define MR_OCCUPANCY __attribute__((amdgpu_waves_per_eu(MR_WAVES_PER_EU, MR_WAVES_PER_EU)))
 #elif defined(MR_VGPRS)
@@ -491,6 +520,14 @@
     const bool rcp_north  = __all(lane > tab_rows || !(0.f >= n_tab));
     const float rcp_tab   = VCACHE ? 0.f : hzf_rcp(rcp_south ? e : hz_abs(n_tab));
 
+#ifdef MR_FACTS_FORCE
+    const uint32_t facts = (uint32_t)(MR_FACTS_FORCE);
+#else
+    const uint32_t facts = mr_strip_facts(p, e, n_tab, jbeg, jend, VCACHE);
+#endif
+    const bool no_far = (facts & HZ_STRIP_NO_FAR_ROWS) != 0;
+    const bool el_unfolded = (facts & HZ_STRIP_EL_UNFOLDED) != 0;
+
     unsigned int head = 0, count = 0;
     if(lane == 0) L.nclip = 0;
     __syncthreads();
@@ -502,7 +539,8 @@
     if(VCACHE) q_next = p.vcache[(size_t)jbeg*p.N + ic];
     float n_cur = north_of(0);
     bool far_prev = true;
-    bool far_cur  = __all(n_cur*n_cur + e*e > p.far_dd);
+    bool far_cur  = false;
+    if(!no_far) { HZF_BRANCH(); far_cur = __all(n_cur*n_cur + e*e > p.far_dd); }
     for(int j = jbeg; j <= jend; j++)
     {
         const int rel = j - jbeg;
@@ -514,7 +552,8 @@
             else z_next = mosaic[(size_t)(j+1)*p.N + ic];
         }
         const float n_next   = (j == jend) ? 0.f : north_of(rel+1);
-        const bool  far_next = (j == jend) || __all(n_next*n_next + e*e > p.far_dd);
+        bool far_next = false;
+        if(!no_far) { HZF_BRANCH(); far_next = (j == jend) || __all(n_next*n_next + e*e > p.far_dd); }
         const bool  skip_row   = far_prev && far_cur && far_next;
         const bool  skip_cells = far_prev && far_cur;
         const float n = n_cur;
@@ -530,7 +569,7 @@
             if(rel >= 64 || !(rcp_south || rcp_north)) rcp_az = hzf_rcp((0.f >= n) ? e : hz_abs(n));
             else if(rcp_south) rcp_az = rcp_tab;
             else rcp_az = __builtin_bit_cast(float, __builtin_amdgcn_readlane(__builtin_bit_cast(int, rcp_tab), rel));
-            vtx = hzf_transform_en_r(&p.u, &fc, e, n, z, rcp_az);
+            vtx = hzf_transform_en_r(&p.u, &fc, e, n, z, rcp_az, el_unfolded);
 #ifdef HZ_EXP_TRANSFORM_TWICE
             {
                 float n2 = n; asm volatile("" : "+v"(n2));
@@ -562,7 +601,7 @@
         if(j > jbeg && !skip_cells)
         {
             bool keep0 = false, keep1 = false;
-            if(cur_simple && prev_simple && mr_simple_cull(prev, now, has_cell, p, &keep0, &keep1))
+            if(cur_simple && prev_simple && mr_simple_cull(prev, now, has_cell, (facts & HZ_STRIP_NARROW_CELLS) != 0, p, &keep0, &keep1))
             {
             }
             else
diff --git a/horizonator_amd/csrc/hz_kernels.hip b/horizonator_amd/csrc/hz_kernels.hip
--- a/horizonator_amd/csrc/hz_kernels.hip
+++ b/horizonator_amd/csrc/hz_kernels.hip
@@ -42,6 +42,20 @@
         }
     }
     mosaic[(size_t)j*N + i] = z;
+}
+
+__global__ __launch_bounds__(256)
+void k_mosaic_range(const int16_t* __restrict__ mosaic, size_t n, int* __restrict__ range)
+{
+    int lo = 32767, hi = -32768;
+    for(size_t k = (size_t)blockIdx.x*blockDim.x + threadIdx.x; k < n; k += (size_t)gridDim.x*blockDim.x)
+    {
+        const int z = mosaic[k];
+        lo = min(lo, z); hi = max(hi, z);
+    }
+    #pragma unroll
+    for(int m=32; m>=1; m>>=1) { lo = min(lo, __shfl_xor(lo, m)); hi = max(hi, __shfl_xor(hi, m)); }
+    if((threadIdx.x & 63) == 0) { atomicMin(&range[0], lo); atomicMax(&range[1], hi); }
 }
 
 
@@ -260,6 +274,11 @@
     hipLaunchKernelGGL(k_ingest, grid, block, 0, stream, tiles, mosaic, N, ntx, nty, cpd, oc_x, oc_y);
 }
 
+void hzk_mosaic_range(dim3 grid, dim3 block, hipStream_t stream, const int16_t* mosaic, size_t n, int* range)
+{
+    hipLaunchKernelGGL(k_mosaic_range, grid, block, 0, stream, mosaic, n, range);
+}
+
 void hzk_link_cells(dim3 grid, dim3 block, hipStream_t stream, const unsigned long long* fb, const float* tanel, const float* sin_az, const float* cos_az, const double* cos_el, float* lat, float* lon, int W, int H, int cell_w, int cell_h, int nx, int ny, float znear, float zfar, double viewer_lat, double cos_viewer_lat, double viewer_lon)
 {
     hipLaunchKernelGGL(k_link_cells, grid, block, 0, stream, fb, tanel, sin_az, cos_az, cos_el, lat, lon, W, H, cell_w, cell_h, nx, ny, znear, zfar, viewer_lat, cos_viewer_lat, viewer_lon);
diff --git a/horizonator_amd/csrc/hz_launch.h b/horizonator_amd/csrc/hz_launch.h
--- a/horizonator_amd/csrc/hz_launch.h
+++ b/horizonator_amd/csrc/hz_launch.h
@@ -22,6 +22,7 @@
 void hzk_tile_bin(dim3 grid, dim3 block, hipStream_t stream, const hz_bigrec_t* bigrec, const hz_bigitem_t* bigitem, const unsigned int* big_counters, unsigned int bigrec_capacity, tl_bins_t tb, hz_params_t p);
 void hzk_tile_raster(dim3 grid, dim3 block, hipStream_t stream, unsigned long long* fb, const hz_bigrec_t* bigrec, tl_bins_t tb, hz_params_t p);
 void hzk_ingest(dim3 grid, dim3 block, hipStream_t stream, const unsigned char* const* tiles, int16_t* mosaic, int N, int ntx, int nty, int cpd, int oc_x, int oc_y);
+void hzk_mosaic_range(dim3 grid, dim3 block, hipStream_t stream, const int16_t* mosaic, size_t n, int* range);
 void hzk_link_cells(dim3 grid, dim3 block, hipStream_t stream, const unsigned long long* fb, const float* tanel, const float* sin_az, const float* cos_az, const double* cos_el, float* lat, float* lon, int W, int H, int cell_w, int cell_h, int nx, int ny, float znear, float zfar, double viewer_lat, double cos_viewer_lat, double viewer_lon);
 void hzk_poi(dim3 grid, dim3 block, hipStream_t stream, const unsigned long long* fb, const float* tanel, const hz_poi_proj_t* proj, int npois, unsigned char* visible, float* label_x, float* label_y, int W, int H, int height_out, float znear, float zfar);
 void hzk_polar_fill(dim3 grid, dim3 block, hipStream_t stream, const int16_t* mosaic, hz_polar_t* q, int N, hz_xform_t u);
diff --git a/horizonator_amd/csrc/hz_plan.cpp b/horizonator_amd/csrc/hz_plan.cpp
--- a/horizonator_amd/csrc/hz_plan.cpp
+++ b/horizonator_amd/csrc/hz_plan.cpp
@@ -89,6 +89,8 @@
 #endif
     p.pretest_march = 0;
     p.fast_ok = hzf_draw_ok(&p.u) && d->env.fast_math;
+    p.z_lo = (float)d->z_lo; p.z_hi = (float)d->z_hi;
+    hz_strip_seam(p.u.az_center, &p.seam_e, &p.seam_n);
     return p;
 }
 
diff --git a/horizonator_amd/csrc/hz_selftest_impl.h b/horizonator_amd/csrc/hz_selftest_impl.h
--- a/horizonator_amd/csrc/hz_selftest_impl.h
+++ b/horizonator_amd/csrc/hz_selftest_impl.h
@@ -258,7 +258,7 @@
         }
         cases++;
         bool keep0 = false, keep1 = false;
-        if(!(simple[0] && simple[1] && mr_simple_cull(st[0], st[1], has_cell, p, &keep0, &keep1))) continue;
+        if(!(simple[0] && simple[1] && mr_simple_cull(st[0], st[1], has_cell, false, p, &keep0, &keep1))) continue;
         shortway++;
         hz_wvert_t v00 = {}, v01 = {}, v10 = {}, v11 = {};
         v00.xn = st[0].xn; v00.xs = st[0].xs; v00.ys = st[0].ys; v00.cmask = st[0].cmask;
@@ -422,6 +422,77 @@
     return (long)items.size();
 }
 
+extern "C" int hz_hip_debug_strip_facts(int N, int W, int H, const hz_view_t* view, const int16_t* mosaic, int z_lo, int z_hi,
+                                        int sx, int jbeg, int jend, int vcache, int32_t* out)
+{
+    if(N < 2 || sx < 0 || sx*MR_COLS >= N || jbeg < 0 || jend < jbeg || jend >= N || jend - jbeg > 64 || !mosaic || !out) return -1;
+    hz_dev_t* d = (hz_dev_t*)calloc(1, sizeof(*d));
+    if(!d) return -1;
+    d->env = hz_options_from_env();
+    d->N = N; d->W = W; d->H = H; d->col0 = 0; d->col1 = W;
+    d->seg_stride = (W + HZ_SEG-1)/HZ_SEG;
+    d->z_lo = z_lo; d->z_hi = z_hi;
+    const hz_params_t p = hz_make_params(d, view);
+    free(d);
+    const int i0 = sx*MR_COLS, nrows = jend - jbeg;
+    float e[64];
+    for(int lane=0; lane<64; lane++) { const int i = i0 + lane; e[lane] = hz_east(&p.u, (float)(i < N ? i : N-1)); }
+    const float n_a = hz_north(&p.u, (float)jbeg), n_b = hz_north(&p.u, (float)jend), e_a = e[0], e_b = e[63];
+    const hz_strip_ext_t x = hz_strip_extent(n_a, n_b, e_a, e_b);
+    uint32_t facts = 0;
+    if(hz_strip_no_far_rows(&x, p.far_dd)) facts |= HZ_STRIP_NO_FAR_ROWS;
+    if(!vcache && hz_strip_el_unfolded(&x, p.z_lo - p.u.viewer_z, p.z_hi - p.u.viewer_z)) facts |= HZ_STRIP_EL_UNFOLDED;
+    const float cell_n = hz_strip_cell_n(&p.u);
+    if(hz_strip_narrow_cells(&x, cell_n*hz_abs(p.u.cos_viewer_lat), cell_n, p.halfW*hz_abs(p.u.az_ndc_per_rad), p.quad_max_dx >> 8))
+    {
+        int all4 = 7, any4 = 0;
+        for(int k=0; k<4; k++) { const int ck = hz_strip_corner((k & 1) ? e_b : e_a, (k & 2) ? n_b : n_a, p.seam_e, p.seam_n); all4 &= ck; any4 |= ck; }
+        if(hz_strip_off_seam(all4, any4)) facts |= HZ_STRIP_NARROW_CELLS;
+    }
+    int32_t far_rows = 0, wide = 0, folded = 0, cells = 0;
+    double az_err = 0.0;
+    int32_t xs[2][64];
+    for(int rel=0; rel<=nrows; rel++)
+    {
+        const float n = hz_north(&p.u, (float)(jbeg + rel));
+        bool all_far = true;
+        int32_t* cur = xs[rel & 1];
+        const int32_t* prev = xs[(rel & 1) ^ 1];
+        for(int lane=0; lane<64; lane++)
+        {
+            const int i = i0 + lane, ic = i < N ? i : N-1;
+            if(!(n*n + e[lane]*e[lane] > p.far_dd)) all_far = false;
+            const float z = (float)mosaic[(size_t)(jbeg + rel)*N + ic];
+            const float h = z - p.u.viewer_z, dne = hz_sqrt(n*n + e[lane]*e[lane]);
+            const float rcp = 1.0f/dne, sot = h*rcp;
+            const float tn = (dne == hz_abs(h)) ? 1.0f : hz_abs(sot);
+            if(1.0f < tn) folded++;
+            if(e[lane] != 0.f || n != 0.f)
+            {
+                double de = fabs((double)hz_atan2(e[lane], n) - atan2((double)e[lane], (double)n));
+                if(de > 3.14159265358979) de = fabs(de - 6.283185307179586);
+                if(de > az_err) az_err = de;
+            }
+            const hz_vertex_t vtx = hz_transform_en(&p.u, e[lane], n, z);
+            const float fxw = (vtx.x*p.halfW + p.halfW) - 0.5f;
+            cur[lane] = (int32_t)hz_roundeven(fxw*256.f);
+        }
+        if(all_far) far_rows++;
+        if(rel > 0)
+            for(int lane=0; lane<MR_COLS; lane++)
+            {
+                if(i0 + lane >= N-1) continue;
+                const int32_t d01x = cur[lane] - prev[lane], d11x = cur[lane+1] - prev[lane], d10x = prev[lane+1] - prev[lane];
+                const int32_t lo = std::min(std::min(d01x, d11x), d10x), hi = std::max(std::max(d01x, d11x), d10x);
+                cells++;
+                if(!(lo > -p.quad_max_dx && hi < p.quad_max_dx)) wide++;
+            }
+    }
+    out[0] = (int32_t)facts; out[1] = far_rows; out[2] = wide; out[3] = folded; out[4] = nrows + 1; out[5] = cells;
+    out[6] = (int32_t)(az_err*1e9 < 2e9 ? az_err*1e9 : 2e9);
+    return 0;
+}
+
 extern "C" int hz_hip_debug_wave_timing(hz_dev_t* d, const hz_view_t* view, unsigned long long* out, size_t capacity_words, unsigned int* grid)
 {
     HZ_ON_DEVICE(d);
diff --git a/horizonator_amd/csrc/hz_strip.h b/horizonator_amd/csrc/hz_strip.h
--- /dev/null
+++ b/horizonator_amd/csrc/hz_strip.h
@@ -0,0 +1,68 @@
+#pragma once
+
+#include <math.h>
+
+#include "hz_num.h"
+
+#define HZ_STRIP_NO_FAR_ROWS   1u
+#define HZ_STRIP_NARROW_CELLS  2u
+#define HZ_STRIP_EL_UNFOLDED   4u
+
+typedef struct
+{
+    float n_lo, n_hi, e_lo, e_hi;
+    float d_lo;
+    int   ok;
+} hz_strip_ext_t;
+
+HZ_HD hz_strip_ext_t hz_strip_extent(float n_a, float n_b, float e_a, float e_b)
+{
+    hz_strip_ext_t x;
+    const float na = hz_abs(n_a), nb = hz_abs(n_b), ea = hz_abs(e_a), eb = hz_abs(e_b);
+    x.ok   = (na <= 3.0e38f && nb <= 3.0e38f && ea <= 3.0e38f && eb <= 3.0e38f) ? 1 : 0;
+    x.n_hi = hz_max(na, nb);
+    x.e_hi = hz_max(ea, eb);
+    x.n_lo = ((n_a > 0.f && n_b > 0.f) || (n_a < 0.f && n_b < 0.f)) ? hz_min(na, nb) : 0.f;
+    x.e_lo = ((e_a > 0.f && e_b > 0.f) || (e_a < 0.f && e_b < 0.f)) ? hz_min(ea, eb) : 0.f;
+    x.d_lo = hz_max(x.n_lo, x.e_lo);
+    return x;
+}
+
+HZ_HD int hz_strip_no_far_rows(const hz_strip_ext_t* x, float far_dd)
+{
+    return x->ok && x->n_hi*x->n_hi + x->e_hi*x->e_hi <= far_dd;
+}
+
+HZ_HD int hz_strip_el_unfolded(const hz_strip_ext_t* x, float h_lo, float h_hi)
+{
+    const float hmax = hz_max(hz_abs(h_lo), hz_abs(h_hi));
+    return x->ok && x->d_lo > 0.f && hz_abs(h_lo) <= 3.0e38f && hz_abs(h_hi) <= 3.0e38f && hmax <= 0.99f*x->d_lo;
+}
+
+HZ_HD float hz_strip_cell_n(const hz_xform_t* u) { return hz_abs(u->deg_per_cell)*111195.0f; }
+
+static inline void hz_strip_seam(float az_center, float* seam_e, float* seam_n)
+{
+    const double a = (double)az_center + 3.14159265358979323846;
+    *seam_e = (float)sin(a); *seam_n = (float)cos(a);
+}
+
+HZ_HD int hz_strip_narrow_cells(const hz_strip_ext_t* x, float cell_e, float cell_n, float px_per_rad, int quad_px)
+{
+    const float L = 1.01f*(cell_e + cell_n) + 1e-6f*(x->e_hi + x->n_hi), D = x->d_lo;
+    return x->ok && quad_px > 0 && L > 0.f && D >= 4.0f*L
+        && 2.0f*((1.02f*L + 4e-4f*D)*px_per_rad + D) <= (float)quad_px*D;
+}
+
+#define HZ_CORNER_CLEAR 1
+#define HZ_CORNER_LEFT  2
+#define HZ_CORNER_AWAY  4
+HZ_HD int hz_strip_corner(float ce, float cn, float seam_e, float seam_n)
+{
+    const float cross = ce*seam_n - cn*seam_e, dot = ce*seam_e + cn*seam_n;
+    return (hz_abs(cross) >= 0.01f*(hz_abs(ce) + hz_abs(cn)) ? HZ_CORNER_CLEAR : 0) | (cross > 0.f ? HZ_CORNER_LEFT : 0) | (dot < 0.f ? HZ_CORNER_AWAY : 0);
+}
+HZ_HD int hz_strip_off_seam(int all4, int any4)
+{
+    return (all4 & HZ_CORNER_CLEAR) && ((all4 & HZ_CORNER_LEFT) || !(any4 & HZ_CORNER_LEFT) || (all4 & HZ_CORNER_AWAY));
+}
diff --git a/horizonator_amd/csrc/hz_types.h b/horizonator_amd/csrc/hz_types.h
--- a/horizonator_amd/csrc/hz_types.h
+++ b/horizonator_amd/csrc/hz_types.h
@@ -4,6 +4,7 @@
 #include <stdint.h>
 
 #include "hz_raster.h"
+#include "hz_strip.h"
 #include "hz_tex.h"
 #include "hz_scatter.h"
 
@@ -44,6 +45,8 @@
     float z_hide_k;
     int   fast_ok;
     int   quad_max_dx;
+    float z_lo, z_hi;
+    float seam_e, seam_n;
 #ifdef HZ_EXPERIMENTS
     int   debug;
 #endif
diff --git a/include/hz_selftest.h b/include/hz_selftest.h
--- a/include/hz_selftest.h
+++ b/include/hz_selftest.h
@@ -17,6 +17,9 @@
 long hz_hip_debug_worklist(int N, int W, int H, const hz_view_t* view, int col0, int col1, int round,
                            int32_t* out, size_t capacity_items);
 
+int  hz_hip_debug_strip_facts(int N, int W, int H, const hz_view_t* view, const int16_t* mosaic, int z_lo, int z_hi,
+                              int sx, int jbeg, int jend, int vcache, int32_t* out);
+
 int  hz_hip_debug_wave_timing(hz_dev_t* d, const hz_view_t* view, unsigned long long* out, size_t capacity_words, unsigned int* grid);
 
 #ifdef __cplusplus
```
